# wyysf-98/MoCo_Flow

Measured on AMD Instinct MI355X. Metric: ray-samples/sec (4096 rays x 64 samples), higher is better.
Workload: dtype f32

## Files before the change

include/mocoflow_hip.h:

```cpp
#ifndef MOCOFLOW_HIP_H
#define MOCOFLOW_HIP_H

#include <stdint.h>

#ifdef __cplusplus
extern "C" {
#endif

#define MF_ABI_VERSION 16

enum {
  MF_OK = 0,
  MF_E_INVALID = -1,
  MF_E_LAUNCH = -2,
  MF_E_UNSUPPORTED = -3
};

enum { MF_MAX_FREQS = 16, MF_MAX_LAYERS = 16 };

enum { MF_PREC_F32 = 0, MF_PREC_BF16 = 1, MF_PREC_BF16X3 = 2 };

typedef struct mf_embedding {
  int32_t in_channels;
  int32_t n_freqs;
  float freq[MF_MAX_FREQS];
  float weight[MF_MAX_FREQS];
} mf_embedding;

enum { MF_EXTRA_NONE = 0, MF_EXTRA_IND = 1, MF_EXTRA_DIR = 2 };

typedef struct mf_nerf_desc {
  int32_t D;
  int32_t W;
  int32_t in_channels_xyz;
  uint32_t skip_mask;
  int32_t extra_feat_type;
  int32_t extra_feat_dim;
  const float* trunk_w[MF_MAX_LAYERS];
  const float* trunk_b[MF_MAX_LAYERS];
  const float* final_w; const float* final_b;
  const float* extra_w; const float* extra_b;
  const float* sigma_w; const float* sigma_b;
  const float* rgb_w;   const float* rgb_b;
} mf_nerf_desc;

typedef struct mf_nof_desc {
  int32_t D;
  int32_t W;
  int32_t in_channels_xyz;
  int32_t extra_feat_dim;
  uint32_t skip_mask;
  int32_t use_quat;
  const float* trunk_w[MF_MAX_LAYERS];
  const float* trunk_b[MF_MAX_LAYERS];
  const float* head_w; const float* head_b;
} mf_nof_desc;

int32_t mf_version(void);
const char* mf_last_error(void);

int64_t mf_nerf_packed_bytes(const mf_nerf_desc* d);
int64_t mf_nof_packed_bytes(const mf_nof_desc* d);
int32_t mf_nerf_pack(const mf_nerf_desc* d, void* packed, void* stream);
int32_t mf_nof_pack(const mf_nof_desc* d, void* packed, void* stream);
int64_t mf_nerf_packed_bytes_p(const mf_nerf_desc* d, int32_t precision);
int64_t mf_nof_packed_bytes_p(const mf_nof_desc* d, int32_t precision);
int32_t mf_nerf_pack_p(const mf_nerf_desc* d, int32_t precision, void* packed, void* stream);
int32_t mf_nof_pack_p(const mf_nof_desc* d, int32_t precision, void* packed, void* stream);

int32_t mf_embedding_forward(const mf_embedding* e, const float* x, int64_t B, float* out, void* stream);
int32_t mf_embedding_forward_rows(const mf_embedding* e, const float* x, int64_t B, int32_t repeat, float* out,
                                  int64_t out_stride, void* stream);

int32_t mf_nerf_forward(const mf_nerf_desc* d, const void* packed, const float* inputs,
                        int64_t in_stride, int64_t B, int32_t sigma_only, float* out, void* stream);

int32_t mf_nerf_forward_dump(const mf_nerf_desc* d, const void* packed, const float* inputs, int64_t in_stride,
                             int64_t B, float* out, float* dump_acts, int64_t dump_stride, void* stream);

int32_t mf_nof_forward(const mf_nof_desc* d, const void* packed, const float* inputs,
                       int64_t in_stride, const float* xyz, int64_t B, float* out, void* stream);

int64_t mf_nerf_bwd_packed_bytes(const mf_nerf_desc* d);
int32_t mf_nerf_pack_bwd(const mf_nerf_desc* d, void* packed, void* stream);
int32_t mf_nerf_backward(const mf_nerf_desc* d, const void* packed_bwd, int64_t P, const float* g_out,
                         const float* acts, int64_t stride, const float* rgbsigma, float* gpre,
                         float* ghead, void* stream);

int32_t mf_nerf_backward_x(const mf_nerf_desc* d, const void* packed_bwd, int64_t P, const float* g_out,
                           const float* acts, int64_t stride, const float* rgbsigma, float* gpre,
                           float* ghead, float* g_emb, void* stream);
int64_t mf_nerf_bwd3_packed_bytes(const mf_nerf_desc* d);
int32_t mf_nerf_pack_bwd3(const mf_nerf_desc* d, void* packed, void* stream);
int32_t mf_nerf_backward3(const mf_nerf_desc* d, const void* packed_bwd3, int64_t P, const float* g_out,
                          const float* acts, int64_t stride, const float* rgbsigma, float* gpre,
                          float* ghead, float* g_emb, const uint32_t* mask, int64_t mask_stride, void* stream);
int32_t mf_embedding_backward(const mf_embedding* e, const float* g_emb, int64_t g_stride, const float* emb,
                              int64_t e_stride, int64_t P, float* g_x, void* stream);

int32_t mf_composite_backward(const float* rays, int64_t ray_stride, int64_t n_rays, int32_t S,
                              const float* z_vals, const float* rgbsigma, const float* noise,
                              int32_t activation, const float* background, const float* g_rgb,
                              const float* g_depth, const float* g_opacity, float* g_rgbsigma, void* stream);

#define MF_WG_MAX_ITEMS 32
typedef struct mf_wgrad_item {
  const float* G; int64_t g_stride; int32_t n_out;
  const float* X; int64_t x_stride; int32_t n_in;
  float* dW; float* db;
} mf_wgrad_item;
int64_t mf_weight_grads_scratch_bytes(const mf_wgrad_item* items, int32_t n_items, int64_t P);
int32_t mf_weight_grads(const mf_wgrad_item* items, int32_t n_items, int64_t P, void* scratch, void* stream);
int64_t mf_weight_grads_scratch_bytes_p(int32_t precision, const mf_wgrad_item* items, int32_t n_items, int64_t P);
int32_t mf_weight_grads_p(int32_t precision, const mf_wgrad_item* items, int32_t n_items, int64_t P, void* scratch, void* stream);

int32_t mf_nof_points_dump(const mf_nof_desc* d, const void* packed, const mf_embedding* emb_xyz,
                           const mf_embedding* emb_ind, const float* pts, const float* ind,
                           int64_t ind_stride, int32_t S, int64_t P, float* out, float* acts,
                           int64_t stride, float* emb, void* stream);
int32_t mf_nof_forward_dump(const mf_nof_desc* d, const void* packed, const float* inputs, int64_t in_stride,
                            const float* xyz, int64_t B, float* out, float* acts, int64_t stride, void* stream);
int64_t mf_nof_bwd_packed_bytes(const mf_nof_desc* d);
int32_t mf_nof_pack_bwd(const mf_nof_desc* d, void* packed, void* stream);
int32_t mf_nof_backward(const mf_nof_desc* d, const void* packed_bwd, const mf_embedding* emb_xyz, int64_t P,
                        const float* pts, const float* acts, int64_t stride, const float* g_out,
                        float* gpre, float* g_pts, void* stream);
int64_t mf_nof_bwd3_packed_bytes(const mf_nof_desc* d);
int32_t mf_nof_pack_bwd3(const mf_nof_desc* d, void* packed, void* stream);
int32_t mf_nof_backward3(const mf_nof_desc* d, const void* packed_bwd3, const mf_embedding* emb_xyz, int64_t P,
                         const float* pts, const float* acts, int64_t stride, const float* g_out,
                         float* gpre, float* g_pts, void* stream);

int32_t mf_points_sigma(const mf_nerf_desc* nerf, const void* nerf_packed, const mf_embedding* emb_xyz,
                        const mf_nof_desc* nof, const void* nof_packed, const mf_embedding* nof_emb_xyz,
                        const mf_embedding* nof_emb_ind, const float* xyz, const float* ind,
                        float ind_scalar, int64_t B, float* sigma, float* canon, void* stream);
int32_t mf_points_sigma_p(int32_t precision, const mf_nerf_desc* nerf, const void* nerf_packed, const mf_embedding* emb_xyz,
                          const mf_nof_desc* nof, const void* nof_packed, const mf_embedding* nof_emb_xyz,
                          const mf_embedding* nof_emb_ind, const float* xyz, const float* ind,
                          float ind_scalar, int64_t B, float* sigma, float* canon, void* workspace,
                          int64_t workspace_bytes, void* stream);
int64_t mf_points_sigma_workspace_bytes(int32_t precision, const mf_nof_desc* nof, int32_t per_point_ind, int64_t B);

int32_t mf_points_radiance(const mf_nerf_desc* nerf, const void* nerf_packed, const mf_embedding* emb_xyz,
                           const mf_embedding* emb_extra, const mf_nof_desc* nof, const void* nof_packed,
                           const mf_embedding* nof_emb_xyz, const mf_embedding* nof_emb_ind, const float* xyz,
                           const float* view_dirs, const float* ind, float ind_scalar, int64_t B, float* out,
                           float* canon, void* stream);

enum {
  MF_ACT_RELU = 0, MF_ACT_SOFTPLUS = 1
};
enum {
  MF_F_SIGMA_ONLY   = 1 << 0,
  MF_F_CHAIN_LOCAL  = 1 << 1,
  MF_F_CHAIN_GLOBAL = 1 << 2
};

typedef struct mf_render_args {
  const float* rays; int64_t ray_stride; int64_t n_rays;
  const float* background;
  int32_t n_samples;
  const float* z_vals; const float* z_steps; int32_t use_disp;
  const float* noise;
  int32_t activation;
  int32_t flags;
  const mf_nerf_desc* nerf; const void* nerf_packed;
  mf_embedding emb_xyz;
  mf_embedding emb_extra;
  const mf_nof_desc* nof_bw; const void* nof_bw_packed;
  const mf_nof_desc* nof_fw; const void* nof_fw_packed;
  mf_embedding nof_emb_xyz, nof_emb_ind;
  float* rgb;
  float* depth;
  float* opacity;
  float* weights;
  float* alphas;
  float* disp_local;
  float* disp_global;
  int32_t precision;
  float* dump_acts; int64_t dump_stride;
  float* dump_rgbsigma;
  float* dump_xyz;
  float* dump_nof_acts; int64_t dump_nof_stride;
  float* dump_nof_emb;
  float* dump_nof_out;
  int32_t dump_nof_plane[5];
  void* workspace; int64_t workspace_bytes;
  uint32_t* dump_mask; int64_t dump_mask_stride;
} mf_render_args;

int32_t mf_render_prepare(const mf_render_args* a, void* stream);
int32_t mf_render_pass(const mf_render_args* a, void* stream);
int64_t mf_render_workspace_bytes(const mf_render_args* a);

int32_t mf_nof_emb_slot_features(int32_t* features80);

int32_t mf_nof_embed_rows(const mf_embedding* emb_xyz, const float* pts, const float* ind_emb, int32_t ind_width, int32_t S,
                          int64_t P, float* out, void* stream);

int32_t mf_sample_pdf(const float* bins, const float* z_coarse, const float* weights, int64_t w_stride,
                      int64_t n_rays, int32_t n_bins, int32_t M, const float* u, int64_t u_stride,
                      const float* cdf_in, float* z_new_out, int32_t* inds_out, float* z_sorted_out,
                      void* stream);
int32_t mf_sample_pdf_eps(const float* bins, const float* z_coarse, const float* weights, int64_t w_stride,
                          int64_t n_rays, int32_t n_bins, int32_t M, const float* u, int64_t u_stride,
                          const float* cdf_in, float* z_new_out, int32_t* inds_out, float* z_sorted_out,
                          float eps, void* stream);
int32_t mf_sample_pdf_merge(const float* z_coarse, const float* weights, int64_t n_rays,
                            int32_t S, int32_t M, const float* u, float* z_out,
                            int32_t* inds_out, float* z_new_out, void* stream);

int64_t mf_compact_scratch_bytes(int64_t n_rays);
int32_t mf_compact_mask(const float* alphas, const float* vals_a, const float* vals_b,
                        int64_t n_rays, int32_t S, float* out_a, float* out_b,
                        int64_t* count, void* scratch, void* stream);

typedef struct mf_loss_pass {
  const float* rgb;
  const float* alphas;
  const float* disp_local;
  const float* disp_global;
  int32_t n_samples;
} mf_loss_pass;
int64_t mf_loss_partials_scratch_bytes(void);
int32_t mf_loss_partials(const mf_loss_pass* coarse, const mf_loss_pass* fine, const float* target, int64_t n_rays,
                         double* out12, float* means6, void* scratch, void* stream);

typedef struct mf_loss_grad_pass {
  const float* rgb; float* g_rgb;
  const float* alphas; int32_t n_samples;
  const float* rays; int64_t ray_stride; const float* z_vals;
  const float* recon_local; float* g_recon_local;
  const float* recon_global; float* g_recon_global;
} mf_loss_grad_pass;
int32_t mf_loss_partials_backward(const mf_loss_grad_pass* coarse, const mf_loss_grad_pass* fine, const float* target,
                                  int64_t n_rays, const double* out12, const double* g12, void* stream);

int32_t mf_z_vals(const float* rays, int64_t ray_stride, int64_t n_rays, const float* z_steps, int32_t n_samples,
                  int32_t use_disp, const float* perturb_rand, float perturb, float* z_out, void* stream);

int32_t mf_make_rays(int32_t H, int32_t W, float focal, float cx, float cy, const float* c2w_host,
                     float nearv, float farv, float idx, float* rays_out, void* stream);
int32_t mf_valid_rays_mask(int32_t H, int32_t W, const int32_t* pts_xy_host, int32_t n_pts, uint8_t* mask_out,
                           void* stream);
int32_t mf_image_compose(const uint8_t* rays_msk, const int64_t* rank, int64_t B, const float* opacity,
                         const float* rgb, const float* depth, const float* background, float* img,
                         float* depth_out, void* stream);

int32_t mf_knn1(const float* ref, int64_t V, const float* query, int64_t Q, float* dist, int64_t* ind,
                void* stream);

typedef struct mf_smpl_model {
  int32_t n_verts;
  const float* v_template;
  const float* shapedirs;
  const float* posedirs;
  const float* j_regressor;
  const float* weights;
  int32_t parent[24];
} mf_smpl_model;

int64_t mf_smpl_scratch_bytes(int64_t n_verts, int64_t B);
int32_t mf_smpl_lbs(const mf_smpl_model* m, const float* pose, int32_t pose_is_rotmat, const float* betas, int64_t B,
                    float* verts, float* T, void* scratch, void* stream);

int32_t mf_smpl_frame_transforms(const float* T_src, const float* T_tgt, int64_t V, float* trans, void* stream);

int32_t mf_apply_vertex_transforms(const float* trans, const int64_t* ind, int64_t V, const float* query, int64_t Q,
                                   float* cano, void* stream);

int64_t mf_mc_scratch_bytes(int64_t n0, int64_t n1, int64_t n2);
int32_t mf_mc_count(const float* vol, int64_t n0, int64_t n1, int64_t n2, float iso, int32_t clamp_zero,
                    void* scratch, int64_t* counts, void* stream);
int32_t mf_mc_emit(const float* vol, int64_t n0, int64_t n1, int64_t n2, float iso, int32_t clamp_zero,
                   const void* scratch, float* verts, int64_t* tris, void* stream);
int32_t mf_mc_normals(const float* vol, int64_t n0, int64_t n1, int64_t n2, int32_t clamp_zero, const float* verts, int64_t V,
                      float* normals, void* stream);

int64_t mf_ssim_scratch_bytes(int64_t B, int64_t C, int64_t H, int64_t W);
int32_t mf_ssim(const float* a, const int64_t* a_strides, const float* b, const int64_t* b_strides, int64_t B, int64_t C,
                int64_t H, int64_t W, int32_t window_size, float max_val, float eps, float* map_out, double* sums,
                void* scratch, void* stream);
int64_t mf_sqerr_scratch_bytes(int64_t n);
int32_t mf_sqerr(const float* a, const float* b, int64_t n, const uint8_t* mask, int64_t row_len, double* out2,
                 void* scratch, void* stream);

int64_t mf_depth_range_scratch_bytes(int64_t n);
int32_t mf_depth_range(const float* depth, int64_t n, float nan_value, float* out2, void* scratch, void* stream);
int32_t mf_depth_colormap(const float* depth, int64_t n, const float* range2, float nan_value, const uint8_t* lut,
                          float* out_planar, void* stream);
typedef struct mf_sheet_panel {
  const float* rows;
  int32_t kind;
  float nan_value;
} mf_sheet_panel;
int32_t mf_frame_sheet(const mf_sheet_panel* panels , int32_t n_panels, int64_t H, int64_t W, const float* range2s,
                       const uint8_t* lut, uint8_t* out_u8, float* out_planar, void* stream);

int64_t mf_mask_compact_scratch_bytes(int64_t n);
int32_t mf_mask_compact(const uint8_t* mask, int64_t n, int64_t* inds_out, int64_t* count, void* scratch, void* stream);

enum { MF_IMAGE_NONE = 0, MF_IMAGE_ROWS = 1, MF_IMAGE_U8_RGB = 2, MF_IMAGE_U8_RGBA = 3 };
enum { MF_BACKGROUND_NONE = 0, MF_BACKGROUND_ROWS = 1, MF_BACKGROUND_COLOUR = 2 };
typedef struct mf_ray_batch_args {
  int32_t H, W;
  float focal, cx, cy;
  int32_t has_c2w; float c2w[12];
  float nearv, farv, idx;
  int32_t has_chain; float chain_idx;
  const int64_t* val_inds; int64_t n_valid;
  const int64_t* perm; int64_t n_rows;
  const void* image; int32_t image_kind;
  const float* background; int32_t background_kind;
  float* rays_out; float* rgbs_out; float* background_out; int64_t* sel_out;
} mf_ray_batch_args;
int32_t mf_ray_batch(const mf_ray_batch_args* a , void* stream);

int32_t mf_point_correspond(const float* verts, const float* trans, int64_t V, const float* query, int64_t q_given,
                            const int64_t* pick, const float* noise, int64_t q_near, float thickness, int32_t lanes_per_query,
                            float* pairs, uint8_t* inside, float* dist, int64_t* ind, void* stream);

typedef struct mf_point_loss_args {
  int64_t Q;
  const float* pairs;
  const uint8_t* inside;
  int32_t use_all;
  const float* pred_bw;
  const float* pred_fw;
  int32_t n_nerfs;
  const float* sigma[2];
  float delta[2];
} mf_point_loss_args;
int64_t mf_point_loss_partials_scratch_bytes(int64_t Q);
int32_t mf_point_loss_partials(const mf_point_loss_args* a , double* out6, float* means3, void* scratch, void* stream);

int32_t mf_point_loss_partials_backward(const mf_point_loss_args* a , const double* out6, const float* seeds3,
                                        float* g_pred_bw, float* g_pred_fw, float* g_sigma0, float* g_sigma1, void* stream);

#ifdef __cplusplus
}
#endif
#endif
```

moco_flow_amd/_lib.py:

```python
from __future__ import annotations

import ctypes as C
import os
import threading

MF_MAX_FREQS = 16
MF_MAX_LAYERS = 16
MF_EXTRA_NONE, MF_EXTRA_IND, MF_EXTRA_DIR = 0, 1, 2
MF_ACT_RELU, MF_ACT_SOFTPLUS = 0, 1
MF_F_SIGMA_ONLY, MF_F_CHAIN_LOCAL, MF_F_CHAIN_GLOBAL = 1, 2, 4
MF_PREC_F32, MF_PREC_BF16, MF_PREC_BF16X3 = 0, 1, 2
PRECISIONS = {"f32": MF_PREC_F32, "bf16": MF_PREC_BF16, "bf16x3": MF_PREC_BF16X3}
MF_ABI_VERSION = 16

LIB_PATH = os.environ.get("MOCOFLOW_HIP_LIB") or os.path.join(os.path.dirname(os.path.abspath(__file__)), "libmocoflow_hip.so")

_fp = C.c_void_p


class mf_embedding(C.Structure):
    _fields_ = [("in_channels", C.c_int32), ("n_freqs", C.c_int32),
                ("freq", C.c_float * MF_MAX_FREQS), ("weight", C.c_float * MF_MAX_FREQS)]


class mf_smpl_model(C.Structure):
    _fields_ = [("n_verts", C.c_int32), ("v_template", _fp), ("shapedirs", _fp), ("posedirs", _fp),
                ("j_regressor", _fp), ("weights", _fp), ("parent", C.c_int32 * 24)]


class mf_nerf_desc(C.Structure):
    _fields_ = [("D", C.c_int32), ("W", C.c_int32), ("in_channels_xyz", C.c_int32),
                ("skip_mask", C.c_uint32), ("extra_feat_type", C.c_int32), ("extra_feat_dim", C.c_int32),
                ("trunk_w", _fp * MF_MAX_LAYERS), ("trunk_b", _fp * MF_MAX_LAYERS),
                ("final_w", _fp), ("final_b", _fp), ("extra_w", _fp), ("extra_b", _fp),
                ("sigma_w", _fp), ("sigma_b", _fp), ("rgb_w", _fp), ("rgb_b", _fp)]


class mf_nof_desc(C.Structure):
    _fields_ = [("D", C.c_int32), ("W", C.c_int32), ("in_channels_xyz", C.c_int32),
                ("extra_feat_dim", C.c_int32), ("skip_mask", C.c_uint32), ("use_quat", C.c_int32),
                ("trunk_w", _fp * MF_MAX_LAYERS), ("trunk_b", _fp * MF_MAX_LAYERS),
                ("head_w", _fp), ("head_b", _fp)]


class mf_wgrad_item(C.Structure):
    _fields_ = [("G", _fp), ("g_stride", C.c_int64), ("n_out", C.c_int32),
                ("X", _fp), ("x_stride", C.c_int64), ("n_in", C.c_int32),
                ("dW", _fp), ("db", _fp)]


MF_WG_MAX_ITEMS = 32


class mf_sheet_panel(C.Structure):
    _fields_ = [("rows", _fp), ("kind", C.c_int32), ("nan_value", C.c_float)]


MF_SHEET_MAX_PANELS = 8
MF_PANEL_RGB, MF_PANEL_DEPTH = 0, 1


MF_IMAGE_NONE, MF_IMAGE_ROWS, MF_IMAGE_U8_RGB, MF_IMAGE_U8_RGBA = 0, 1, 2, 3
MF_BACKGROUND_NONE, MF_BACKGROUND_ROWS, MF_BACKGROUND_COLOUR = 0, 1, 2


class mf_ray_batch_args(C.Structure):
    _fields_ = [("H", C.c_int32), ("W", C.c_int32), ("focal", C.c_float), ("cx", C.c_float), ("cy", C.c_float),
                ("has_c2w", C.c_int32), ("c2w", C.c_float * 12), ("nearv", C.c_float), ("farv", C.c_float), ("idx", C.c_float),
                ("has_chain", C.c_int32), ("chain_idx", C.c_float),
                ("val_inds", _fp), ("n_valid", C.c_int64), ("perm", _fp), ("n_rows", C.c_int64),
                ("image", _fp), ("image_kind", C.c_int32), ("background", _fp), ("background_kind", C.c_int32),
                ("rays_out", _fp), ("rgbs_out", _fp), ("background_out", _fp), ("sel_out", _fp)]


class mf_point_loss_args(C.Structure):
    _fields_ = [("Q", C.c_int64), ("pairs", _fp), ("inside", _fp), ("use_all", C.c_int32), ("pred_bw", _fp), ("pred_fw", _fp),
                ("n_nerfs", C.c_int32), ("sigma", _fp * 2), ("delta", C.c_float * 2)]


class mf_loss_pass(C.Structure):
    _fields_ = [("rgb", _fp), ("alphas", _fp), ("disp_local", _fp), ("disp_global", _fp), ("n_samples", C.c_int32)]


class mf_loss_grad_pass(C.Structure):
    _fields_ = [("rgb", _fp), ("g_rgb", _fp), ("alphas", _fp), ("n_samples", C.c_int32),
                ("rays", _fp), ("ray_stride", C.c_int64), ("z_vals", _fp),
                ("recon_local", _fp), ("g_recon_local", _fp), ("recon_global", _fp), ("g_recon_global", _fp)]


class mf_render_args(C.Structure):
    _fields_ = [("rays", _fp), ("ray_stride", C.c_int64), ("n_rays", C.c_int64),
                ("background", _fp), ("n_samples", C.c_int32),
                ("z_vals", _fp), ("z_steps", _fp), ("use_disp", C.c_int32),
                ("noise", _fp), ("activation", C.c_int32), ("flags", C.c_int32),
                ("nerf", C.POINTER(mf_nerf_desc)), ("nerf_packed", _fp),
                ("emb_xyz", mf_embedding), ("emb_extra", mf_embedding),
                ("nof_bw", C.POINTER(mf_nof_desc)), ("nof_bw_packed", _fp),
                ("nof_fw", C.POINTER(mf_nof_desc)), ("nof_fw_packed", _fp),
                ("nof_emb_xyz", mf_embedding), ("nof_emb_ind", mf_embedding),
                ("rgb", _fp), ("depth", _fp), ("opacity", _fp), ("weights", _fp), ("alphas", _fp),
                ("disp_local", _fp), ("disp_global", _fp), ("precision", C.c_int32),
                ("dump_acts", _fp), ("dump_stride", C.c_int64), ("dump_rgbsigma", _fp), ("dump_xyz", _fp),
                ("dump_nof_acts", _fp), ("dump_nof_stride", C.c_int64), ("dump_nof_emb", _fp), ("dump_nof_out", _fp),
                ("dump_nof_plane", C.c_int32 * 5),
                ("workspace", _fp), ("workspace_bytes", C.c_int64),
                ("dump_mask", _fp), ("dump_mask_stride", C.c_int64)]


SYMBOLS = {
    "mf_version": (C.c_int32, []),
    "mf_last_error": (C.c_char_p, []),
    "mf_nerf_packed_bytes": (C.c_int64, [C.POINTER(mf_nerf_desc)]),
    "mf_nof_packed_bytes": (C.c_int64, [C.POINTER(mf_nof_desc)]),
    "mf_nerf_pack": (C.c_int32, [C.POINTER(mf_nerf_desc), _fp, _fp]),
    "mf_nof_pack": (C.c_int32, [C.POINTER(mf_nof_desc), _fp, _fp]),
    "mf_nerf_packed_bytes_p": (C.c_int64, [C.POINTER(mf_nerf_desc), C.c_int32]),
    "mf_nof_packed_bytes_p": (C.c_int64, [C.POINTER(mf_nof_desc), C.c_int32]),
    "mf_nerf_pack_p": (C.c_int32, [C.POINTER(mf_nerf_desc), C.c_int32, _fp, _fp]),
    "mf_nof_pack_p": (C.c_int32, [C.POINTER(mf_nof_desc), C.c_int32, _fp, _fp]),
    "mf_embedding_forward": (C.c_int32, [C.POINTER(mf_embedding), _fp, C.c_int64, _fp, _fp]),
    "mf_embedding_forward_rows": (C.c_int32, [C.POINTER(mf_embedding), _fp, C.c_int64, C.c_int32, _fp, C.c_int64, _fp]),
    "mf_nerf_forward": (C.c_int32, [C.POINTER(mf_nerf_desc), _fp, _fp, C.c_int64, C.c_int64, C.c_int32, _fp, _fp]),
    "mf_nerf_forward_dump": (C.c_int32, [C.POINTER(mf_nerf_desc), _fp, _fp, C.c_int64, C.c_int64, _fp, _fp, C.c_int64, _fp]),
    "mf_nof_forward": (C.c_int32, [C.POINTER(mf_nof_desc), _fp, _fp, C.c_int64, _fp, C.c_int64, _fp, _fp]),
    "mf_nerf_bwd_packed_bytes": (C.c_int64, [C.POINTER(mf_nerf_desc)]),
    "mf_nerf_pack_bwd": (C.c_int32, [C.POINTER(mf_nerf_desc), _fp, _fp]),
    "mf_nof_points_dump": (C.c_int32, [C.POINTER(mf_nof_desc), _fp, C.POINTER(mf_embedding), C.POINTER(mf_embedding), _fp, _fp,
                                       C.c_int64, C.c_int32, C.c_int64, _fp, _fp, C.c_int64, _fp, _fp]),
    "mf_nof_forward_dump": (C.c_int32, [C.POINTER(mf_nof_desc), _fp, _fp, C.c_int64, _fp, C.c_int64, _fp, _fp, C.c_int64, _fp]),
    "mf_nof_bwd_packed_bytes": (C.c_int64, [C.POINTER(mf_nof_desc)]),
    "mf_nof_pack_bwd": (C.c_int32, [C.POINTER(mf_nof_desc), _fp, _fp]),
    "mf_nof_backward": (C.c_int32, [C.POINTER(mf_nof_desc), _fp, C.POINTER(mf_embedding), C.c_int64, _fp, _fp, C.c_int64,
                                    _fp, _fp, _fp, _fp]),
    "mf_nof_backward3": (C.c_int32, [C.POINTER(mf_nof_desc), _fp, C.POINTER(mf_embedding), C.c_int64, _fp, _fp, C.c_int64,
                                    _fp, _fp, _fp, _fp]),
    "mf_nof_bwd3_packed_bytes": (C.c_int64, [C.POINTER(mf_nof_desc)]),
    "mf_nof_pack_bwd3": (C.c_int32, [C.POINTER(mf_nof_desc), _fp, _fp]),
    "mf_composite_backward": (C.c_int32, [_fp, C.c_int64, C.c_int64, C.c_int32, _fp, _fp, _fp, C.c_int32, _fp, _fp, _fp, _fp,
                                          _fp, _fp]),
    "mf_image_compose": (C.c_int32, [_fp, _fp, C.c_int64, _fp, _fp, _fp, _fp, _fp, _fp, _fp]),
    "mf_weight_grads_scratch_bytes": (C.c_int64, [C.POINTER(mf_wgrad_item), C.c_int32, C.c_int64]),
    "mf_weight_grads": (C.c_int32, [C.POINTER(mf_wgrad_item), C.c_int32, C.c_int64, _fp, _fp]),
    "mf_weight_grads_scratch_bytes_p": (C.c_int64, [C.c_int32, C.POINTER(mf_wgrad_item), C.c_int32, C.c_int64]),
    "mf_weight_grads_p": (C.c_int32, [C.c_int32, C.POINTER(mf_wgrad_item), C.c_int32, C.c_int64, _fp, _fp]),
    "mf_nerf_bwd3_packed_bytes": (C.c_int64, [C.POINTER(mf_nerf_desc)]),
    "mf_nerf_pack_bwd3": (C.c_int32, [C.POINTER(mf_nerf_desc), _fp, _fp]),
    "mf_nerf_backward3": (C.c_int32, [C.POINTER(mf_nerf_desc), _fp, C.c_int64, _fp, _fp, C.c_int64, _fp, _fp, _fp, _fp, _fp, C.c_int64, _fp]),
    "mf_nerf_backward": (C.c_int32, [C.POINTER(mf_nerf_desc), _fp, C.c_int64, _fp, _fp, C.c_int64, _fp, _fp, _fp, _fp]),
    "mf_render_pass": (C.c_int32, [C.POINTER(mf_render_args), _fp]),
    "mf_render_workspace_bytes": (C.c_int64, [C.POINTER(mf_render_args)]),
    "mf_render_prepare": (C.c_int32, [C.POINTER(mf_render_args), _fp]),
    "mf_points_sigma_workspace_bytes": (C.c_int64, [C.c_int32, C.POINTER(mf_nof_desc), C.c_int32, C.c_int64]),
    "mf_points_sigma": (C.c_int32, [C.POINTER(mf_nerf_desc), _fp, C.POINTER(mf_embedding), C.POINTER(mf_nof_desc), _fp,
                                    C.POINTER(mf_embedding), C.POINTER(mf_embedding), _fp, _fp, C.c_float, C.c_int64,
                                    _fp, _fp, _fp]),
    "mf_points_sigma_p": (C.c_int32, [C.c_int32, C.POINTER(mf_nerf_desc), _fp, C.POINTER(mf_embedding), C.POINTER(mf_nof_desc), _fp,
                                      C.POINTER(mf_embedding), C.POINTER(mf_embedding), _fp, _fp, C.c_float, C.c_int64,
                                      _fp, _fp, _fp, C.c_int64, _fp]),
    "mf_points_radiance": (C.c_int32, [C.POINTER(mf_nerf_desc), _fp, C.POINTER(mf_embedding), C.POINTER(mf_embedding),
                                       C.POINTER(mf_nof_desc), _fp, C.POINTER(mf_embedding), C.POINTER(mf_embedding), _fp, _fp,
                                       _fp, C.c_float, C.c_int64, _fp, _fp, _fp]),
    "mf_sample_pdf_merge": (C.c_int32, [_fp, _fp, C.c_int64, C.c_int32, C.c_int32, _fp, _fp, _fp, _fp, _fp]),
    "mf_sample_pdf": (C.c_int32, [_fp, _fp, _fp, C.c_int64, C.c_int64, C.c_int32, C.c_int32, _fp, C.c_int64,
                                  _fp, _fp, _fp, _fp, _fp]),
    "mf_sample_pdf_eps": (C.c_int32, [_fp, _fp, _fp, C.c_int64, C.c_int64, C.c_int32, C.c_int32, _fp, C.c_int64,
                                      _fp, _fp, _fp, _fp, C.c_float, _fp]),
    "mf_z_vals": (C.c_int32, [_fp, C.c_int64, C.c_int64, _fp, C.c_int32, C.c_int32, _fp, C.c_float, _fp, _fp]),
    "mf_make_rays": (C.c_int32, [C.c_int32, C.c_int32, C.c_float, C.c_float, C.c_float, C.POINTER(C.c_float),
                                 C.c_float, C.c_float, C.c_float, _fp, _fp]),
    "mf_knn1": (C.c_int32, [_fp, C.c_int64, _fp, C.c_int64, _fp, _fp, _fp]),
    "mf_nof_emb_slot_features": (C.c_int32, [C.POINTER(C.c_int32)]),
    "mf_nof_embed_rows": (C.c_int32, [C.POINTER(mf_embedding), _fp, _fp, C.c_int32, C.c_int32, C.c_int64, _fp, _fp]),
    "mf_smpl_scratch_bytes": (C.c_int64, [C.c_int64, C.c_int64]),
    "mf_smpl_lbs": (C.c_int32, [C.POINTER(mf_smpl_model), _fp, C.c_int32, _fp, C.c_int64, _fp, _fp, _fp, _fp]),
    "mf_smpl_frame_transforms": (C.c_int32, [_fp, _fp, C.c_int64, _fp, _fp]),
    "mf_apply_vertex_transforms": (C.c_int32, [_fp, _fp, C.c_int64, _fp, C.c_int64, _fp, _fp]),
    "mf_nerf_backward_x": (C.c_int32, [C.POINTER(mf_nerf_desc), _fp, C.c_int64, _fp, _fp, C.c_int64, _fp, _fp, _fp, _fp, _fp]),
    "mf_embedding_backward": (C.c_int32, [C.POINTER(mf_embedding), _fp, C.c_int64, _fp, C.c_int64, C.c_int64, _fp, _fp]),
    "mf_valid_rays_mask": (C.c_int32, [C.c_int32, C.c_int32, C.POINTER(C.c_int32), C.c_int32, _fp, _fp]),
    "mf_loss_partials_scratch_bytes": (C.c_int64, []),
    "mf_loss_partials": (C.c_int32, [C.POINTER(mf_loss_pass), C.POINTER(mf_loss_pass), _fp, C.c_int64, _fp, _fp, _fp, _fp]),
    "mf_loss_partials_backward": (C.c_int32, [C.POINTER(mf_loss_grad_pass), C.POINTER(mf_loss_grad_pass), _fp, C.c_int64, _fp, _fp, _fp]),
    "mf_compact_scratch_bytes": (C.c_int64, [C.c_int64]),
    "mf_compact_mask": (C.c_int32, [_fp, _fp, _fp, C.c_int64, C.c_int32, _fp, _fp, _fp, _fp, _fp]),
    "mf_mc_scratch_bytes": (C.c_int64, [C.c_int64, C.c_int64, C.c_int64]),
    "mf_mc_count": (C.c_int32, [_fp, C.c_int64, C.c_int64, C.c_int64, C.c_float, C.c_int32, _fp, _fp, _fp]),
    "mf_mc_emit": (C.c_int32, [_fp, C.c_int64, C.c_int64, C.c_int64, C.c_float, C.c_int32, _fp, _fp, _fp, _fp]),
    "mf_mc_normals": (C.c_int32, [_fp, C.c_int64, C.c_int64, C.c_int64, C.c_int32, _fp, C.c_int64, _fp, _fp]),
    "mf_ssim_scratch_bytes": (C.c_int64, [C.c_int64, C.c_int64, C.c_int64, C.c_int64]),
    "mf_ssim": (C.c_int32, [_fp, C.POINTER(C.c_int64), _fp, C.POINTER(C.c_int64), C.c_int64, C.c_int64, C.c_int64, C.c_int64,
                            C.c_int32, C.c_float, C.c_float, _fp, _fp, _fp, _fp]),
    "mf_sqerr_scratch_bytes": (C.c_int64, [C.c_int64]),
    "mf_sqerr": (C.c_int32, [_fp, _fp, C.c_int64, _fp, C.c_int64, _fp, _fp, _fp]),
    "mf_depth_range_scratch_bytes": (C.c_int64, [C.c_int64]),
    "mf_depth_range": (C.c_int32, [_fp, C.c_int64, C.c_float, _fp, _fp, _fp]),
    "mf_depth_colormap": (C.c_int32, [_fp, C.c_int64, _fp, C.c_float, _fp, _fp, _fp]),
    "mf_frame_sheet": (C.c_int32, [C.POINTER(mf_sheet_panel), C.c_int32, C.c_int64, C.c_int64, _fp, _fp, _fp, _fp, _fp]),
    "mf_mask_compact_scratch_bytes": (C.c_int64, [C.c_int64]),
    "mf_mask_compact": (C.c_int32, [_fp, C.c_int64, _fp, _fp, _fp, _fp]),
    "mf_ray_batch": (C.c_int32, [C.POINTER(mf_ray_batch_args), _fp]),
    "mf_point_correspond": (C.c_int32, [_fp, _fp, C.c_int64, _fp, C.c_int64, _fp, _fp, C.c_int64, C.c_float, C.c_int32,
                                        _fp, _fp, _fp, _fp, _fp]),
    "mf_point_loss_partials_scratch_bytes": (C.c_int64, [C.c_int64]),
    "mf_point_loss_partials": (C.c_int32, [C.POINTER(mf_point_loss_args), _fp, _fp, _fp, _fp]),
    "mf_point_loss_partials_backward": (C.c_int32, [C.POINTER(mf_point_loss_args), _fp, _fp, _fp, _fp, _fp, _fp, _fp]),
}

_lock = threading.Lock()
_lib = None


def lib():
    global _lib
    if _lib is not None:
        return _lib
    with _lock:
        if _lib is None:
            if not os.path.exists(LIB_PATH):
                raise RuntimeError(
                    f"moco_flow_amd: HIP library not built ({LIB_PATH} missing). "
                    "Run `make -C moco_flow_amd/csrc` (hipcc, gfx950). There is no CPU fallback.")
            handle = C.CDLL(LIB_PATH)
            for name, (res, args) in SYMBOLS.items():
                fn = getattr(handle, name)
                fn.restype = res
                fn.argtypes = args
            if handle.mf_version() != MF_ABI_VERSION:
                raise RuntimeError("moco_flow_amd: ABI version mismatch")
            _lib = handle
    return _lib


def check(rc: int, what: str = ""):
    if rc != 0:
        msg = lib().mf_last_error().decode(errors="replace")
        if rc == -3:
            raise NotImplementedError(f"moco_flow_amd HIP path: {msg}")
        raise RuntimeError(f"moco_flow_amd HIP call failed ({what}, rc={rc}): {msg}")


def ptr(t):
    return None if t is None else t.data_ptr()


def current_stream(device) -> int:
    import torch
    return torch.cuda.current_stream(device).cuda_stream


def require_gpu(t, what: str):
    if not t.is_cuda:
        raise RuntimeError(
            f"moco_flow_amd.{what}: tensor is on '{t.device}'. This package is the MI355X (HIP) path and has "
            "no CPU implementation; move the module and its inputs to a 'cuda' device.")
```

moco_flow_amd/csrc/mf_layout.hpp:

```cpp
#pragma once
#include "../../include/mocoflow_hip.h"
#include "mf_core.hpp"

namespace mf {

inline int64_t round_up(int64_t x, int64_t m) { return (x + m - 1) / m * m; }

inline int single_skip_layer(uint32_t skip_mask, int D) {
  int s = 0;
  for (int l = 1; l < D; ++l)
    if ((skip_mask >> l) & 1u) { if (s) return -1; s = l; }
  return s;
}

constexpr int kPackHidden = -1;
struct PackBlock {
  const float* src;
  int s_n, s_k;
  int kind;
  int steps;
  int split;
  int cols;
};

struct PackRegion {
  PackBlock blk[2];
  int tiles;
  int groups;
  int n_rows;
  int row_terms;
  long long dst_group0;
};

struct ResCopy { const float* src; int dst_off; int n; float scale = 1.f; };

struct PackJob {
  PackRegion reg[MF_MAX_LAYERS + 3];
  int n_regions;
  int bf16;
  int xyz_cols;
  int half;
  float wscale;
  long long total_groups;
  float* panels;
  float* poison;
  ResCopy res[2];
  int n_res, res_floats;
  float* resident;
  PackRegion& add(int tiles, int groups, const PackBlock& b0, const PackBlock& b1 = PackBlock{}) {
    PackRegion& R = reg[n_regions++];
    R = PackRegion{{b0, b1}, tiles, groups, 0, 0, total_groups};
    total_groups += (long long)groups * tiles;
    return R;
  }
};
static_assert(sizeof(PackJob) <= 2048, "pack_panels_kernel's argument block");

int launch_pack(const PackJob& job, hipStream_t st, const char* what);

inline bool nerf_layout(const mf_nerf_desc& d, NetLayout& L, int bf16 = 0) {
  L = NetLayout{};
  const bool x3 = bf16 == MF_PREC_BF16X3;
  L.bf16 = bf16 ? 1 : 0;
  if (d.W != 256 && d.W != 128) return false;
  if (d.D < 2 || d.D + 1 > MF_MAX_LAYERS) return false;
  if (d.in_channels_xyz < 3 || d.in_channels_xyz > 64) return false;
  if (d.extra_feat_type != MF_EXTRA_NONE && (d.extra_feat_dim < 1 || d.extra_feat_dim > 32)) return false;
  if (d.skip_mask & 1u) return false;
  if (d.skip_mask >> d.D) return false;
  L.W = d.W;
  L.NK = d.W / 16;
  L.NP = d.W / 32;
  L.n_trunk = d.D + 1;
  if (bf16 && d.W != 256) return false;
  L.emb_steps = bf16 ? kKsNerfXyz : kStepsNerfXyz;
  L.emb_split = x3 ? 1 : 0;
  L.hsplit_mask = x3 ? ((1u << (d.D + 2)) - 1u) & ~1u : 0u;
  L.terms = 2;
  L.emb_mask = 1u | d.skip_mask;
  L.relu_mask = (1u << d.D) - 1u;
  switch (d.extra_feat_type) {
    case MF_EXTRA_NONE: L.extra_steps = 0; break;
    case MF_EXTRA_IND: L.extra_steps = bf16 ? kKsInd : kStepsInd; if (d.extra_feat_dim < 1) return false; break;
    case MF_EXTRA_DIR: L.extra_steps = bf16 ? kKsDir : kStepsDir; if (d.extra_feat_dim < 3) return false; break;
    default: return false;
  }
  int off = 0;
  L.off_bias_trunk = off; off += L.n_trunk * L.W;
  L.off_bias_extra = off; off += L.W / 2;
  L.off_head_w = off; off += L.W;
  L.off_head_b = off; off += 4;
  L.off_rgb_w = off; off += 3 * (L.W / 2);
  L.off_rgb_b = off; off += 4;
  L.n_head = 1;
  L.head_tiles = bf16 == MF_PREC_BF16 ? 1 : 0;
  L.res_bytes = round_up((int64_t)off * 4, kGroupBytes);
  int64_t groups = 0;
  L.max_groups = 0;
  for (int l = 0; l < L.n_trunk; ++l) {
    if (l == L.n_trunk - 1) groups += nerf_sigma_groups(L);
    const int g = trunk_groups(L, l);
    groups += (int64_t)g * L.NP;
    if ((x3 ? panel_cap(g) : g) > L.max_groups) L.max_groups = x3 ? panel_cap(g) : g;
  }
  const int ge = extra_groups(L);
  groups += (int64_t)ge * (L.NP / 2);
  if ((x3 ? panel_cap(ge) : ge) > L.max_groups) L.max_groups = x3 ? panel_cap(ge) : ge;
  groups += nerf_rgb_groups(L);
  L.panel_bytes = groups * kGroupBytes;
  return true;
}

inline bool nof_layout(const mf_nof_desc& d, NetLayout& L, int bf16 = 0, bool wide_ok = false) {
  L = NetLayout{};
  const bool x3 = bf16 == MF_PREC_BF16X3;
  L.bf16 = bf16 ? 1 : 0;
  if (d.W != 128 && !(wide_ok && !bf16 && d.W == 256)) return false;
  if (d.D < 2 || d.D > MF_MAX_LAYERS) return false;
  if (d.in_channels_xyz < 3 || d.in_channels_xyz > 33 || d.extra_feat_dim < 0 || d.extra_feat_dim > 33) return false;
  if ((d.skip_mask & 1u) || (d.skip_mask >> d.D)) return false;
  L.W = d.W;
  L.NK = d.W / 16;
  L.NP = d.W / 32;
  L.n_trunk = d.D;
  L.emb_steps = bf16 ? kKsNofXyz : kStepsNofIn;
  L.emb_split = bf16 ? 1 : 0;
  L.hsplit_mask = x3 ? ((1u << d.D) - 1u) & ~1u : 0u;
  L.terms = x3 ? kNofTermsX3 : 2;
  L.half = (x3 && kNofHalfX3) ? 1 : 0;
  L.head_tiles = bf16 == MF_PREC_BF16 ? 1 : 0;
  L.emb_mask = 1u | d.skip_mask;
  L.relu_mask = (1u << d.D) - 1u;
  L.extra_steps = -1;
  L.n_head = d.use_quat ? 9 : 3;
  int off = 0;
  L.off_bias_trunk = off; off += L.n_trunk * L.W;
  L.off_head_w = off; off += L.n_head * L.W;
  L.off_head_b = off; off += bf16 ? 32 : 12;
  L.res_bytes = round_up((int64_t)off * 4, kGroupBytes);
  int64_t groups = 0;
  L.max_groups = 0;
  for (int l = 0; l < L.n_trunk; ++l) {
    const int g = trunk_groups(L, l);
    groups += (int64_t)g * L.NP;
    if ((x3 ? panel_cap(g) : g) > L.max_groups) L.max_groups = x3 ? panel_cap(g) : g;
  }
  if (bf16) {
    groups += head_groups(L);
    if (head_groups(L) > L.max_groups) L.max_groups = head_groups(L);
  }
  L.panel_bytes = groups * kGroupBytes;
  L.n_emb_layers = __builtin_popcount(L.emb_mask);
  L.ind_bytes = bf16 ? round_up((int64_t)L.n_emb_layers * L.W * kNofIndCols * 4, kGroupBytes) : 0;
  return true;
}

}
```

moco_flow_amd/csrc/mf_nets.hpp:

```cpp
#pragma once
#include "mf_core.hpp"

namespace mf {

MF_D const char* first_panel(const NetDev& n) { return n.packed + n.L.res_bytes; }
MF_D int first_groups(const NetDev& n) { return trunk_groups(n.L, 0); }

MF_D NextLayer follow_of(const NetDev& n) {
  NextLayer f;
  f.groups = trunk_groups(n.L, 0);
  f.jump = n.packed + n.L.res_bytes;
  f.bias_off = n.res_lds + n.L.off_bias_trunk * 4;
  return f;
}
MF_D NextLayer next_trunk(const NetDev& n, int layer) {
  NextLayer f;
  f.groups = trunk_groups(n.L, layer);
  f.jump = nullptr;
  f.bias_off = n.res_lds + (n.L.off_bias_trunk + layer * n.L.W) * 4;
  return f;
}

MF_D void load_resident(const NetDev& n, const LaneId& id) {
  const int groups = (int)(n.L.res_bytes / kGroupBytes);
  for (int g = id.wave; g < groups; g += kWaves) blds16(n.packed, id.lane * 16, g * kGroupBytes, n.res_lds + g * kGroupBytes);
}

template <int PD>
MF_D void start_program(const NetDev& n, Stream& st, CarryT<PD>& carry, const LaneId& id) {
  st.start(first_panel(n), first_groups(n), id);
  carry.load(st.slot_off(0) + id.lane * 16, n.res_lds + n.L.off_bias_trunk * 4, id.g);
}

template <int NK, bool DUMP = false>
MF_D void extra_layer(const NetDev& net, const f32x4 (&act)[NK],
                      const float (&ext)[kStepsExtraMax], f32x4 (&out)[NK / 2],
                      Stream& st, CarryT<kPD>& carry, const LaneId& id, const NextLayer& nxt,
                      float* dump_row = nullptr, unsigned* mask_row = nullptr) {
  constexpr int NPO = NK / 4;
  constexpr int QH = NK;
  const int groups = extra_groups(net.L);
  const int qe = net.L.extra_steps / 4;
  const uint32_t bias_off = net.res_lds + net.L.off_bias_extra * 4;
  const float dummy[4] = {0.f, 0.f, 0.f, 0.f};
  static_assert(NPO % 4 == 0, "mask words collect four panels");
  unsigned macc = 0;
#pragma unroll
  for (int t = 0; t < NPO; ++t) {
    const uint32_t p = st.slot_off(0) + id.lane * 16;
    const uint32_t pn = st.slot_off(1) + id.lane * 16;
    const uint32_t nb = (t + 1 < NPO) ? bias_off + 32 * (t + 1) * 4 : nxt.bias_off;
    auto hook = [&](int ph) { st.template sync_and_dma<DUMP>(t + 2 < NPO ? groups : nxt.groups, t == NPO - 2 ? nxt.jump : nullptr, id, ph); };
    f32x4 E, O;
    out_pair<2, NK, 4>(carry, act, dummy, p, pn, nb, id.g, id.wave < kWaves / 2 && !(st.dbg & 64), hook,
                             -__builtin_inff(), E, O);
#pragma unroll
    for (int q = 0; q < kStepsExtraMax / 4; ++q) {
      if (q < qe) {
        const f32x4 wE = lds_f4(p + (2 * (QH + q)) * kGroupBytes);
        const f32x4 wO = lds_f4(p + (2 * (QH + q) + 1) * kGroupBytes);
#pragma unroll
        for (int r = 0; r < 4; ++r) {
          E = MF_MFMA(wE[r], ext[4 * q + r], E);
          O = MF_MFMA(wO[r], ext[4 * q + r], O);
        }
      }
    }
#pragma unroll
    for (int i = 0; i < 4; ++i) {
      E[i] = fmaxf(E[i], 0.f);
      O[i] = fmaxf(O[i], 0.f);
    }
    out[2 * t] = E;
    out[2 * t + 1] = O;
    if constexpr (DUMP) {
      if (dump_row) {
        *reinterpret_cast<f32x4*>(dump_row + 32 * t + 4 * id.g) = E;
        *reinterpret_cast<f32x4*>(dump_row + 32 * t + 16 + 4 * id.g) = O;
      }
      const bool wm = __ballot(mask_row != nullptr) != 0ull;
      const bool put = wm && relu_mask_put(macc, mask_row, dump_row && mask_row, t, id.g, E, O);
      st.keep2 = __ballot(dump_row != nullptr) != 0ull ? (put ? 3 : 2) : 0;
    }
    st.advance();
  }
}

template <int NK, bool DUMP = false>
MF_D void nerf_eval(const NetDev& net, const float (&embx)[kStepsNerfXyz], const float (&ext)[kStepsExtraMax],
                    bool sigma_only, Stream& st, CarryT<kPD>& carry, const LaneId& id,
                    const NextLayer& follow, float& sigma, float (&rgb)[3], float* dump_row = nullptr,
                    unsigned* mask_row = nullptr) {
  f32x4 act[NK];
#pragma unroll
  for (int t = 0; t < NK; ++t)
#pragma unroll
    for (int i = 0; i < 4; ++i) act[t][i] = 0;
  const int D = net.L.n_trunk - 1;
  for (int l = 0; l < D; ++l) {
    const bool last = sigma_only && l == D - 1;
    trunk_layer<NK, kStepsNerfXyz, DUMP>(net, l, act, embx, st, carry, id, last ? follow : next_trunk(net, l + 1),
                                               dump_row ? dump_row + l * net.L.W : nullptr, mask_row ? mask_row + l * 8 : nullptr);
    st.tl.stamp(10 + l, id);
  }
  float sg[1];
  valu_head(act, net.res_lds + net.L.off_head_w * 4, net.L.W, net.res_lds + net.L.off_head_b * 4, id.g, sg);
  sigma = sg[0];
  st.tl.stamp(30, id);
  if (sigma_only) return;
  NextLayer ex;
  ex.groups = extra_groups(net.L);
  ex.jump = nullptr;
  ex.bias_off = net.res_lds + net.L.off_bias_extra * 4;
  trunk_layer<NK, kStepsNerfXyz, DUMP>(net, D, act, embx, st, carry, id, ex,
                                             dump_row ? dump_row + D * net.L.W : nullptr);
  st.tl.stamp(31, id);
  f32x4 e[NK / 2];
  extra_layer<NK, DUMP>(net, act, ext, e, st, carry, id, follow, dump_row ? dump_row + (D + 1) * net.L.W : nullptr,
                        mask_row ? mask_row + (D + 1) * 8 : nullptr);
  st.tl.stamp(33, id);
  float o[3];
  valu_head(e, net.res_lds + net.L.off_rgb_w * 4, net.L.W / 2, net.res_lds + net.L.off_rgb_b * 4, id.g, o);
#pragma unroll
  for (int c = 0; c < 3; ++c) rgb[c] = 1.f / (1.f + expf(-o[c]));
}

template <bool FAST = false>
MF_D void quat_transform(const float (&T)[9], const float (&xyz)[3], float (&out)[3]) {
  const float vx = T[0], vy = T[1], vz = T[2];
  float qx, qy, qz, qw;
  if constexpr (FAST) {
    const float n = fmaxf(__builtin_amdgcn_sqrtf(vx * vx + vy * vy + vz * vz), 1e-8f);
    const float rev = n * 0.15915494309189535f;
    const float s_n = __builtin_amdgcn_sinf(rev) * __builtin_amdgcn_rcpf(n);
    qx = vx * s_n; qy = vy * s_n; qz = vz * s_n; qw = __builtin_amdgcn_cosf(rev);
    const float rq = __builtin_amdgcn_rcpf(fmaxf(__builtin_amdgcn_sqrtf(qx * qx + qy * qy + qz * qz + qw * qw), 1e-12f));
    qx *= rq; qy *= rq; qz *= rq; qw *= rq;
  } else {
    float n = sqrtf(vx * vx + vy * vy + vz * vz);
    n = fmaxf(n, 1e-8f);
    float sn, cn;
    sincosf(n, &sn, &cn);
    qx = vx * sn / n; qy = vy * sn / n; qz = vz * sn / n; qw = cn;
    const float qn = fmaxf(sqrtf(qx * qx + qy * qy + qz * qz + qw * qw), 1e-12f);
    qx /= qn; qy /= qn; qz /= qn; qw /= qn;
  }
  const float tx = 2.f * qx, ty = 2.f * qy, tz = 2.f * qz;
  const float twx = tx * qw, twy = ty * qw, twz = tz * qw;
  const float txx = tx * qx, txy = ty * qx, txz = tz * qx;
  const float tyy = ty * qy, tyz = tz * qy, tzz = tz * qz;
  const float R00 = 1.f - (tyy + tzz), R01 = txy - twz, R02 = txz + twy;
  const float R10 = txy + twz, R11 = 1.f - (txx + tzz), R12 = tyz - twx;
  const float R20 = txz - twy, R21 = tyz + twx, R22 = 1.f - (txx + tyy);
  const float px = xyz[0] - T[3], py = xyz[1] - T[4], pz = xyz[2] - T[5];
  out[0] = (px * R00 + py * R10 + pz * R20) + T[3] + T[6];
  out[1] = (px * R01 + py * R11 + pz * R21) + T[4] + T[7];
  out[2] = (px * R02 + py * R12 + pz * R22) + T[5] + T[8];
}

template <bool DUMP = false, int NK = 8>
MF_D void nof_eval(const NetDev& net, const float (&emb)[kStepsNofIn], const float (&xyz)[3], Stream& st,
                   CarryT<kPD>& carry, const LaneId& id, const NextLayer& follow, float (&out)[3],
                   float* drow = nullptr, bool masks = false) {
  static_assert(!DUMP || NK == 8, "the dump layout (bit rows: four words per layer) is the 128-wide one");
  f32x4 act[NK];
#pragma unroll
  for (int t = 0; t < NK; ++t)
#pragma unroll
    for (int i = 0; i < 4; ++i) act[t][i] = 0;
  const int D = net.L.n_trunk;
  for (int l = 0; l < D; ++l) {
    const bool last = l == D - 1;
    trunk_layer<NK, kStepsNofIn, DUMP>(net, l, act, emb, st, carry, id, last ? follow : next_trunk(net, l + 1),
                                       drow ? drow + l * net.L.W : nullptr,
                                       (DUMP && drow && masks) ? reinterpret_cast<unsigned*>(drow + D * net.L.W + 16) + 4 * l : nullptr);
  }
  const uint32_t wo = net.res_lds + net.L.off_head_w * 4, bo = net.res_lds + net.L.off_head_b * 4;
  float T[9] = {0.f, 0.f, 0.f, 0.f, 0.f, 0.f, 0.f, 0.f, 0.f};
  if (net.L.n_head == 9) {
    valu_head(act, wo, net.L.W, bo, id.g, T);
    quat_transform(T, xyz, out);
  } else {
    float T3[3];
    valu_head(act, wo, net.L.W, bo, id.g, T3);
#pragma unroll
    for (int c = 0; c < 3; ++c) { T[c] = T3[c]; out[c] = T3[c] + xyz[c]; }
  }
  if constexpr (DUMP) {
    if (drow && id.g == 0) {
      float4* tr = reinterpret_cast<float4*>(drow + D * net.L.W);
      tr[0] = make_float4(T[0], T[1], T[2], T[3]);
      tr[1] = make_float4(T[4], T[5], T[6], T[7]);
      tr[2] = make_float4(T[8], 0.f, 0.f, 0.f);
      tr[3] = make_float4(0.f, 0.f, 0.f, 0.f);
    }
  }
}

MF_D void nof_embed(float (&emb)[kStepsNofIn], const float (&xyz)[3], float ind, const EmbParams& exyz,
                    const EmbParams& eind, int g) {
  emb_eval<3, 5>(emb, xyz, exyz, g);
  const float iv[1] = {ind};
  emb_eval<1, 16>(emb + BlkXyz5::SLOTS, iv, eind, g);
#pragma unroll
  for (int e = BlkXyz5::SLOTS + BlkInd16::SLOTS; e < kStepsNofIn; ++e) emb[e] = 0.f;
}

MF_D void nof_embed_lds(float (&emb)[kStepsNofIn], const float (&xyz)[3], float ind, uint32_t par_xyz, uint32_t par_ind, int g) {
  emb_eval_lds<3, 5>(emb, xyz, par_xyz, g);
  const float iv[1] = {ind};
  emb_eval_lds<1, 16>(emb + BlkXyz5::SLOTS, iv, par_ind, g);
#pragma unroll
  for (int e = BlkXyz5::SLOTS + BlkInd16::SLOTS; e < kStepsNofIn; ++e) emb[e] = 0.f;
}

}
```

moco_flow_amd/csrc/mf_pack.hip:

```cpp
#include <hip/hip_fp16.h>
#include "mf_host.hpp"
#include "mf_layout.hpp"

namespace mf {

__device__ inline unsigned short bf16_rne(float x) {
  const unsigned u = __float_as_uint(x);
  const unsigned rnd = u + 0x7fffu + ((u >> 16) & 1u);
  return (unsigned short)(((u & 0x7f800000u) == 0x7f800000u ? u : rnd) >> 16);
}

__device__ inline float resident_value(const ResCopy* c, int n, int idx) {
  float v = 0.f;
  for (int k = 0; k < n; ++k) {
    const int o = idx - c[k].dst_off;
    if (o >= 0 && o < c[k].n) v = c[k].src[o] * c[k].scale;
  }
  return v;
}

__device__ inline float block_at(const PackBlock& B, int n, int c) {
  return (c >= 0 && c < B.cols) ? B.src[(long long)n * B.s_n + (long long)c * B.s_k] : 0.f;
}

__global__ void pack_panels_kernel(PackJob job) {
  const long long gidx = (long long)blockIdx.x * blockDim.x + threadIdx.x;
  if (gidx < job.res_floats) job.resident[gidx] = resident_value(job.res, job.n_res, (int)gidx);
  const long long grp = ((long long)blockIdx.x * blockDim.x + __builtin_amdgcn_readfirstlane(threadIdx.x)) >> 6;
  if (grp >= job.total_groups) return;
  const int lane = (int)(gidx & 63);
  int ri = 0;
  while (ri + 1 < job.n_regions && grp >= job.reg[ri + 1].dst_group0) ++ri;
  const PackRegion& R = job.reg[ri];
  const long long local = grp - R.dst_group0;
  const int P = (int)(local / R.groups), gi = (int)(local % R.groups);
  float4 v = make_float4(0.f, 0.f, 0.f, 0.f);
  float* pv = &v.x;
  if (job.bf16) {
    const int i = lane & 31, h = lane >> 5;
    int srow = 32 * P + i, rterm = 0;
    bool zero_row = R.n_rows && srow >= R.n_rows;
    if (R.row_terms) {
      zero_row = !(srow < R.n_rows || (srow >= R.row_terms && srow < R.row_terms + R.n_rows));
      if (srow >= R.row_terms) { rterm = 1; srow -= R.row_terms; }
    }
    const int g0 = R.blk[0].split * R.blk[0].steps;
    const PackBlock B = gi < g0 ? R.blk[0] : R.blk[1];
    const int gb = gi < g0 ? gi : gi - g0;
    unsigned short h8[8] = {0, 0, 0, 0, 0, 0, 0, 0};
    const bool half = job.half != 0;
    const float ws = job.wscale;
    bool sat = false;
    auto term = [half, ws, &sat](float w, int t) {
      if (half) {
        w = w * ws;
        if (!(fabsf(w) <= 65504.f)) sat = true;
        w = fminf(fmaxf(w, -65504.f), 65504.f);
        __half hb = __float2half_rn(w);
        if (t > 0) hb = __float2half_rn(w - __half2float(hb));
        return __half_as_ushort(hb);
      }
      unsigned short b = bf16_rne(w);
      for (int k = 0; k < t; ++k) {
        w -= __uint_as_float((unsigned)b << 16);
        b = bf16_rne(w);
      }
      return b;
    };
    if (!zero_row && gb < B.split * B.steps) {
      const int ks = gb / B.split, t = R.row_terms ? rterm : gb % B.split;
#pragma unroll
      for (int e = 0; e < 8; ++e) {
        const int c = B.kind == kPackHidden ? 16 * ks + hid_perm2(h, e) : emb_feature2(B.kind, h, 8 * ks + e, job.xyz_cols);
        h8[e] = term(block_at(B, srow, c), t);
      }
    }
    unsigned* pu = reinterpret_cast<unsigned*>(&v.x);
    for (int w = 0; w < 4; ++w) pu[w] = (unsigned)h8[2 * w] | ((unsigned)h8[2 * w + 1] << 16);
    reinterpret_cast<float4*>(job.panels)[gidx] = v;
    if (sat && job.poison) { job.poison[0] = __int_as_float(0x7fc00000); job.poison[4] = __int_as_float(0x7fc00000); }
    return;
  }
  const int b = gi >> 1, half = gi & 1;
  const int i = lane & 15, g = lane >> 4;
  const int n = 32 * P + 16 * half + i;
  const PackBlock B = b < R.blk[0].steps ? R.blk[0] : R.blk[1];
  const int q = b < R.blk[0].steps ? b : b - R.blk[0].steps;
  if (!(R.n_rows && n >= R.n_rows) && q < B.steps)
#pragma unroll
    for (int r = 0; r < 4; ++r)
      pv[r] = block_at(B, n, B.kind == kPackHidden ? 16 * q + 4 * g + r : emb_feature(B.kind, g, 4 * q + r, job.xyz_cols));
  reinterpret_cast<float4*>(job.panels)[gidx] = v;
}

struct ResJob { ResCopy c[2 * MF_MAX_LAYERS + 8]; int n; float* res; int total; };

__global__ void pack_resident_kernel(ResJob job) {
  const int idx = blockIdx.x * blockDim.x + threadIdx.x;
  if (idx >= job.total) return;
  job.res[idx] = resident_value(job.c, job.n, idx);
}

struct IndJob { const float* W[MF_MAX_LAYERS]; int n_in[MF_MAX_LAYERS]; int n_layers, rows, col0, cols; float* dst; float scale; };

__global__ void pack_ind_kernel(IndJob job) {
  const int idx = blockIdx.x * blockDim.x + threadIdx.x;
  const int per_layer = job.rows * kNofIndCols;
  if (idx >= job.n_layers * per_layer) return;
  const int e = idx / per_layer, r = (idx % per_layer) / kNofIndCols, c = idx % kNofIndCols;
  job.dst[(e * kNofIndCols + c) * job.rows + r] = c < job.cols ? job.scale * job.W[e][(long long)r * job.n_in[e] + job.col0 + c] : 0.f;
}

int launch_pack(const PackJob& job, hipStream_t st, const char* what) {
  const long long slots = job.total_groups * 64 > job.res_floats ? job.total_groups * 64 : job.res_floats;
  hipLaunchKernelGGL(pack_panels_kernel, dim3((unsigned)((slots + 255) / 256)), dim3(256), 0, st, job);
  return check_launch(what);
}

static int launch_pack(const PackJob& job, const ResJob& rj, hipStream_t st) {
  hipLaunchKernelGGL(pack_resident_kernel, dim3((rj.total + 255) / 256), dim3(256), 0, st, rj);
  return launch_pack(job, st, "mf_pack");
}

}

using namespace mf;

extern "C" int64_t mf_nerf_packed_bytes_p(const mf_nerf_desc* d, int32_t precision) {
  NetLayout L;
  if (!d || (precision < MF_PREC_F32 || precision > MF_PREC_BF16X3) || !nerf_layout(*d, L, precision)) { fail(MF_E_UNSUPPORTED, "mf_nerf_packed_bytes: unsupported NeRF configuration"); return 0; }
  return L.res_bytes + L.panel_bytes;
}

extern "C" int64_t mf_nof_packed_bytes_p(const mf_nof_desc* d, int32_t precision) {
  NetLayout L;
  if (!d || (precision < MF_PREC_F32 || precision > MF_PREC_BF16X3) || !nof_layout(*d, L, precision, precision == MF_PREC_F32)) { fail(MF_E_UNSUPPORTED, "mf_nof_packed_bytes: unsupported NoF configuration"); return 0; }
  return L.res_bytes + L.panel_bytes + L.ind_bytes;
}

extern "C" int32_t mf_nerf_pack_p(const mf_nerf_desc* d, int32_t precision, void* packed, void* stream) {
  NetLayout L;
  if (!d || !packed) return fail(MF_E_INVALID, "mf_nerf_pack: null argument");
  if (precision < MF_PREC_F32 || precision > MF_PREC_BF16X3) return fail(MF_E_INVALID, "mf_nerf_pack: precision %d", precision);
  if (!nerf_layout(*d, L, precision)) return fail(MF_E_UNSUPPORTED, "mf_nerf_pack: unsupported NeRF configuration "
                                       "(W=%d D=%d in_channels_xyz=%d)", d->W, d->D, d->in_channels_xyz);
  PackJob job{};
  ResJob rj{};
  const int esplit = L.emb_split ? L.terms : 1, equad = L.bf16 ? 1 : 4;
  auto head_region = [&](const float* W, int rows, int groups) {
    PackRegion& R = job.add(1, groups, PackBlock{W, groups * 16, 1, kPackHidden, groups, 1, groups * 16});
    R.n_rows = rows;
    R.row_terms = 8;
  };
  for (int l = 0; l < L.n_trunk; ++l) {
    if (l == L.n_trunk - 1 && L.head_tiles) {
      if (!d->sigma_w) return fail(MF_E_INVALID, "mf_nerf_pack: missing sigma weight");
      head_region(d->sigma_w, 1, nerf_sigma_groups(L));
    }
    const bool has_emb = (L.emb_mask >> l) & 1;
    const float* W = l < d->D ? d->trunk_w[l] : d->final_w;
    if (!W) return fail(MF_E_INVALID, "mf_nerf_pack: missing weight pointer for layer %d", l);
    const int hid0 = has_emb ? d->in_channels_xyz : 0, n_in = hid0 + (l > 0 ? L.W : 0);
    job.add(L.NP, trunk_groups(L, l),
            PackBlock{W, n_in, 1, kEmbNerfXyz, has_emb ? L.emb_steps / equad : 0, esplit, d->in_channels_xyz},
            PackBlock{W + hid0, n_in, 1, kPackHidden, l > 0 ? hidden_batches(L) : 0, ((L.hsplit_mask >> l) & 1) ? L.terms : 1, L.W});
    const float* b = l < d->D ? d->trunk_b[l] : d->final_b;
    rj.c[rj.n++] = ResCopy{b, L.off_bias_trunk + l * L.W, L.W};
  }
  {
    const int ext = d->extra_feat_type == MF_EXTRA_NONE ? 0 : d->extra_feat_dim;
    const float* W = d->extra_w;
    if (!W) return fail(MF_E_INVALID, "mf_nerf_pack: missing extra_encoding weight");
    const int kind = d->extra_feat_type == MF_EXTRA_DIR ? kEmbDir : (d->extra_feat_type == MF_EXTRA_IND ? kEmbInd : kEmbNone);
    job.add(L.NP / 2, extra_groups(L),
            PackBlock{W, L.W + ext, 1, kPackHidden, hidden_batches(L), ((L.hsplit_mask >> L.n_trunk) & 1) ? L.terms : 1, L.W},
            PackBlock{W + L.W, L.W + ext, 1, kind, L.extra_steps / equad, esplit, ext});
    rj.c[rj.n++] = ResCopy{d->extra_b, L.off_bias_extra, L.W / 2};
  }
  if (L.head_tiles) {
    if (!d->rgb_w) return fail(MF_E_INVALID, "mf_nerf_pack: missing rgb weight");
    head_region(d->rgb_w, 3, nerf_rgb_groups(L));
  }
  rj.c[rj.n++] = ResCopy{d->sigma_w, L.off_head_w, L.W};
  rj.c[rj.n++] = ResCopy{d->sigma_b, L.off_head_b, 1};
  rj.c[rj.n++] = ResCopy{d->rgb_w, L.off_rgb_w, 3 * (L.W / 2)};
  rj.c[rj.n++] = ResCopy{d->rgb_b, L.off_rgb_b, 3};
  for (int k = 0; k < rj.n; ++k)
    if (!rj.c[k].src) return fail(MF_E_INVALID, "mf_nerf_pack: missing bias/head pointer (%d)", k);
  job.bf16 = L.bf16;
  job.xyz_cols = d->in_channels_xyz;
  job.panels = reinterpret_cast<float*>(static_cast<char*>(packed) + L.res_bytes);
  rj.res = static_cast<float*>(packed);
  rj.total = (int)(L.res_bytes / 4);
  if (job.total_groups * kGroupBytes != L.panel_bytes) return fail(MF_E_INVALID, "mf_nerf_pack: layout mismatch");
  return launch_pack(job, rj, static_cast<hipStream_t>(stream));
}

extern "C" int32_t mf_nof_pack_p(const mf_nof_desc* d, int32_t precision, void* packed, void* stream) {
  NetLayout L;
  if (!d || !packed) return fail(MF_E_INVALID, "mf_nof_pack: null argument");
  if (precision < MF_PREC_F32 || precision > MF_PREC_BF16X3) return fail(MF_E_INVALID, "mf_nof_pack: precision %d", precision);
  if (!nof_layout(*d, L, precision, precision == MF_PREC_F32)) return fail(MF_E_UNSUPPORTED, "mf_nof_pack: unsupported NoF configuration "
                                      "(W=%d D=%d in_channels_xyz=%d extra_feat_dim=%d)", d->W, d->D,
                                      d->in_channels_xyz, d->extra_feat_dim);
  PackJob job{};
  ResJob rj{};
  const int cin = d->in_channels_xyz + d->extra_feat_dim;
  const float wscale = L.half ? (float)(1 << kNofHalfSW) : 1.f, bscale = L.half ? (float)(1 << (kNofHalfSA + kNofHalfSW)) : 1.f;
  const int esplit = L.emb_split ? L.terms : 1, equad = L.bf16 ? 1 : 4;
  for (int l = 0; l < L.n_trunk; ++l) {
    const bool has_emb = (L.emb_mask >> l) & 1;
    const float* W = d->trunk_w[l];
    if (!W || !d->trunk_b[l]) return fail(MF_E_INVALID, "mf_nof_pack: missing parameter pointer for layer %d", l);
    const int hid0 = has_emb ? cin : 0, n_in = hid0 + (l > 0 ? L.W : 0);
    job.add(L.NP, trunk_groups(L, l),
            PackBlock{W, n_in, 1, kEmbNofIn, has_emb ? L.emb_steps / equad : 0, esplit, cin},
            PackBlock{W + hid0, n_in, 1, kPackHidden, l > 0 ? hidden_batches(L) : 0, ((L.hsplit_mask >> l) & 1) ? L.terms : 1, L.W});
    rj.c[rj.n++] = ResCopy{d->trunk_b[l], L.off_bias_trunk + l * L.W, L.W, bscale};
  }
  if (!d->head_w || !d->head_b) return fail(MF_E_INVALID, "mf_nof_pack: missing head parameters");
  if (L.bf16) {
    PackRegion& R = job.add(1, head_groups(L), PackBlock{d->head_w, L.W, 1, kPackHidden, L.NK, L.head_tiles ? 1 : L.terms, L.W});
    R.n_rows = L.n_head;
    R.row_terms = L.head_tiles ? 16 : 0;
  }
  rj.c[rj.n++] = ResCopy{d->head_w, L.off_head_w, L.n_head * L.W};
  rj.c[rj.n++] = ResCopy{d->head_b, L.off_head_b, L.n_head, bscale};
  job.bf16 = L.bf16;
  job.xyz_cols = d->in_channels_xyz;
  job.half = L.half;
  job.wscale = wscale;
  job.panels = reinterpret_cast<float*>(static_cast<char*>(packed) + L.res_bytes);
  job.poison = L.half ? static_cast<float*>(packed) + L.off_head_b + 27 : nullptr;
  rj.res = static_cast<float*>(packed);
  rj.total = (int)(L.res_bytes / 4);
  if (job.total_groups * kGroupBytes != L.panel_bytes) return fail(MF_E_INVALID, "mf_nof_pack: layout mismatch");
  if (L.bf16) {
    IndJob ij{};
    for (int l = 0; l < L.n_trunk; ++l)
      if ((L.emb_mask >> l) & 1) {
        ij.W[ij.n_layers] = d->trunk_w[l];
        ij.n_in[ij.n_layers] = cin + (l > 0 ? L.W : 0);
        ++ij.n_layers;
      }
    ij.rows = L.W; ij.col0 = d->in_channels_xyz; ij.cols = d->extra_feat_dim;
    ij.scale = bscale;
    ij.dst = reinterpret_cast<float*>(static_cast<char*>(packed) + L.res_bytes + L.panel_bytes);
    const int total = ij.n_layers * ij.rows * kNofIndCols;
    hipLaunchKernelGGL(pack_ind_kernel, dim3((total + 255) / 256), dim3(256), 0, static_cast<hipStream_t>(stream), ij);
  }
  return launch_pack(job, rj, static_cast<hipStream_t>(stream));
}

extern "C" int64_t mf_nerf_packed_bytes(const mf_nerf_desc* d) { return mf_nerf_packed_bytes_p(d, MF_PREC_F32); }
extern "C" int64_t mf_nof_packed_bytes(const mf_nof_desc* d) { return mf_nof_packed_bytes_p(d, MF_PREC_F32); }
extern "C" int32_t mf_nerf_pack(const mf_nerf_desc* d, void* packed, void* stream) { return mf_nerf_pack_p(d, MF_PREC_F32, packed, stream); }
extern "C" int32_t mf_nof_pack(const mf_nof_desc* d, void* packed, void* stream) { return mf_nof_pack_p(d, MF_PREC_F32, packed, stream); }
```

moco_flow_amd/csrc/mf_render.hip:

```cpp
#include <cstddef>

#include "mf_host.hpp"
#include "mf_layout.hpp"
#include "mf_nets.hpp"
#include "mf_plan.hpp"
#include "mf_raypass.hpp"

namespace mf {

struct RenderParams {
  const float* rays; long long ray_stride; long long n_rays;
  const float* bg;
  int S;
  const float* z_vals; const float* z_steps; int use_disp;
  const float* noise;
  int activation, flags;
  NetDev nerf;
  int extra_type;
  NetDev bw, fw;
  float emb_par[4][32];
  uint32_t par_off;
  float *rgb, *depth, *opacity, *weights, *alphas, *disp_local, *disp_global;
  int G;
  long long n_groups;
  uint32_t ring_off, buf_bytes, sbuf_off, zbuf_off;
  int dbg;
  float* dump_acts; long long dump_stride; float* dump_rgbsigma; float* dump_xyz;
  unsigned* dump_mask; long long dump_mask_stride;
  float* dump_nof_acts; long long dump_nof_stride; float* dump_nof_emb; float* dump_nof_out;
  uint32_t nof_plane_pack;
};

template <bool MOCO, bool DUMP>
__global__ __launch_bounds__(kThreads, 2) void render_kernel(RenderParams p) {
  const LaneId id;
  const NetDev nerf = p.nerf;
  const WgClock wg;
  load_resident(nerf, id);
  if (MOCO) {
    load_resident(p.bw, id);
    if (p.flags & (MF_F_CHAIN_LOCAL | MF_F_CHAIN_GLOBAL)) load_resident(p.fw, id);
  }
  emb_tables_to_lds(p);
  const uint32_t par_nerf_xyz = p.par_off, par_nerf_ext = p.par_off + 128, par_nof_xyz = p.par_off + 256,
                 par_nof_ind = p.par_off + 384;
  Stream st;
  CarryT<kPD> carry;
  st.open(p.ring_off, p.buf_bytes, MF_TIMING_FLAGS ? p.dbg : 0);
  st.tl.start(p.alphas, id);
  const NextLayer prog_first = MOCO ? follow_of(p.bw) : follow_of(nerf);
  if (MOCO) start_program(p.bw, st, carry, id);
  else start_program(nerf, st, carry, id);

  const int S = p.S;
  const bool sigma_only = p.flags & MF_F_SIGMA_ONLY;
  float4* sbuf = reinterpret_cast<float4*>(smem + p.sbuf_off);
  float* zbuf = reinterpret_cast<float*>(smem + p.zbuf_off);

  for (long long group = blockIdx.x; group < p.n_groups; group += gridDim.x) {
    const long long ray0 = group * p.G;
    const int nr = (int)((p.n_rays - ray0) < p.G ? (p.n_rays - ray0) : p.G);
    const int nsamp = nr * S;
    const int ntiles = (nsamp + kTile - 1) / kTile;

    for (int tile = 0; tile < ntiles; ++tile) {
      st.tl.stamp(1, id);
      struct Where { int srel, sl, si; bool valid; long long ray; const float* rp; };
      auto where = [&]() {
        int jo = id.j;
        asm volatile("" : "+v"(jo));
        Where w;
        w.srel = tile * kTile + id.wave * kWaveSamples + jo;
        w.valid = w.srel < nsamp;
        w.sl = w.valid ? w.srel : nsamp - 1;
        const int rr = w.sl / S;
        w.si = w.sl - rr * S;
        w.ray = ray0 + rr;
        w.rp = p.rays + w.ray * p.ray_stride;
        return w;
      };
      float xin[3];
      {
        const Where w = where();
        const float* rp = w.rp;
        const float o[3] = {rp[0], rp[1], rp[2]};
        const float d[3] = {rp[3], rp[4], rp[5]};
        const float z = ray_depth(p, rp, w.ray, w.si);
        ray_point(o, d, z, xin);
        if (w.valid && id.g == 0) {
          zbuf[w.srel] = z;
          if (MOCO) sbuf[w.srel] = make_float4(xin[0], xin[1], xin[2], 0.f);
        }
      }
#ifdef MF_TIMELINE
      asm volatile("s_waitcnt vmcnt(0)" : "+v"(xin[0]), "+v"(xin[1]), "+v"(xin[2]));
#endif
      st.tl.stamp(2, id);
      if (MOCO) {
        const int nsteps = chain_steps(p.flags);
        float canon[3] = {0.f, 0.f, 0.f}, cur[3] = {xin[0], xin[1], xin[2]};
        for (int step = 0; step < nsteps; ++step) {
          const int role = step;
          const NetDev net = role_uses_fw(role) ? p.fw : p.bw;
          const Where w = where();
          const float ind = w.rp[role_ind_column(role)];
          if (role == 1 || role == 2) { cur[0] = canon[0]; cur[1] = canon[1]; cur[2] = canon[2]; }
          const bool last = step == nsteps - 1;
          const NextLayer follow = last ? follow_of(nerf) : (role_uses_fw(role + 1) ? follow_of(p.fw) : follow_of(p.bw));
          float emb[kStepsNofIn], out[3];
          nof_embed_lds(emb, cur, ind, par_nof_xyz, par_nof_ind, id.g);
          float* nof_row = nullptr;
          if constexpr (DUMP) {
            if (w.valid && p.dump_nof_acts) {
              const long long nof_idx = (long long)((p.nof_plane_pack >> (3 * step)) & 7u) * p.n_rays * S + (w.ray * S + w.si);
              nof_row = p.dump_nof_acts + nof_idx * p.dump_nof_stride;
              float4* e4 = reinterpret_cast<float4*>(p.dump_nof_emb + nof_idx * 80 + 20 * id.g);
#pragma unroll
              for (int q = 0; q < kStepsNofIn / 4; ++q) e4[q] = make_float4(emb[4 * q], emb[4 * q + 1], emb[4 * q + 2], emb[4 * q + 3]);
            }
            st.keep2 = 0;
          }
          nof_eval<DUMP>(net, emb, cur, st, carry, id, follow, out, nof_row,
                         DUMP && p.dump_nof_stride >= (long long)net.L.n_trunk * net.L.W + 16 + 4 * net.L.n_trunk);
          if constexpr (DUMP) {
            const Where v = where();
            if (v.valid && p.dump_nof_acts && id.g == 0) {
              const long long nof_idx = (long long)((p.nof_plane_pack >> (3 * step)) & 7u) * p.n_rays * S + (v.ray * S + v.si);
              float* q = p.dump_nof_out + nof_idx * 3;
              q[0] = out[0]; q[1] = out[1]; q[2] = out[2];
            }
          }
          if (role == 0) { canon[0] = out[0]; canon[1] = out[1]; canon[2] = out[2]; }
          if (role == 1 || role == 4) {
            const Where v = where();
            const float4 x4 = sbuf[v.sl];
            const float dd = (fabsf(x4.x - out[0]) + fabsf(x4.y - out[1]) + fabsf(x4.z - out[2])) / 3.f;
            float* plane = role == 1 ? p.disp_local : p.disp_global;
            if (v.valid && id.g == 0 && plane) plane[v.ray * S + v.si] = dd;
          }
          cur[0] = out[0]; cur[1] = out[1]; cur[2] = out[2];
        }
        xin[0] = canon[0]; xin[1] = canon[1]; xin[2] = canon[2];
      }

      st.tl.stamp(3, id);
      float embx[kStepsNerfXyz], ext[kStepsExtraMax];
      if (!(MF_TIMING_FLAGS && (p.dbg & 4))) emb_eval_lds<3, 10>(embx, xin, par_nerf_xyz, id.g);
      else { for (int e = 0; e < kStepsNerfXyz; ++e) embx[e] = xin[e % 3]; }
#pragma unroll
      for (int e = BlkXyz10::SLOTS; e < kStepsNerfXyz; ++e) embx[e] = 0.f;
#pragma unroll
      for (int e = 0; e < kStepsExtraMax; ++e) ext[e] = 0.f;
      float* dump_row = nullptr;
      unsigned* mask_row = nullptr;
      {
        const Where w = where();
        if (!sigma_only) {
          if (p.extra_type == MF_EXTRA_DIR) {
            const float dd[3] = {w.rp[3], w.rp[4], w.rp[5]};
            emb_eval_lds<3, 4>(ext, dd, par_nerf_ext, id.g);
          } else if (p.extra_type == MF_EXTRA_IND) {
            const float iv[1] = {w.rp[8]};
            emb_eval_lds<1, 2>(ext, iv, par_nerf_ext, id.g);
          }
        }
        if constexpr (DUMP) {
          if (w.valid && p.dump_acts) dump_row = p.dump_acts + (w.ray * S + w.si) * p.dump_stride;
          if (p.dump_mask) mask_row = p.dump_mask + (w.ray * S + w.si) * p.dump_mask_stride;
        }
      }
      st.tl.stamp(4, id);
      float sigma, rgb[3] = {0.f, 0.f, 0.f};
      st.keep2 = 0;
      nerf_eval<16, DUMP>(nerf, embx, ext, sigma_only, st, carry, id, prog_first, sigma, rgb, dump_row, mask_row);
      {
        const Where w = where();
        if (w.valid && id.g == 0) {
          sbuf[w.srel] = make_float4(rgb[0], rgb[1], rgb[2], sigma);
          if constexpr (DUMP) {
            const long long row = w.ray * S + w.si;
            if (p.dump_rgbsigma) *reinterpret_cast<float4*>(p.dump_rgbsigma + row * 4) = make_float4(rgb[0], rgb[1], rgb[2], sigma);
            if (p.dump_xyz) { float* q = p.dump_xyz + row * 3; q[0] = xin[0]; q[1] = xin[1]; q[2] = xin[2]; }
          }
        }
      }
      st.tl.stamp(5, id);
    }
    __syncthreads();
    st.tl.stamp(6, id);

    composite_group<kWaves>(p, id.lane, id.wave, ray0, (MF_TIMING_FLAGS && (p.dbg & 8)) ? 0 : nr, S, sigma_only, sbuf, zbuf);
    st.tl.stamp(7, id);
    __syncthreads();
    st.tl.stamp(8, id);
  }
  wait_vm0();
  wg.stamp(p);
}

int render_pass_bf16(const mf_render_args* a, hipStream_t st, bool prepare_only);
int64_t render_workspace_bytes_bf16(const mf_render_args* a);

}

using namespace mf;

extern "C" int64_t mf_render_workspace_bytes(const mf_render_args* a) {
  if (!a || (a->precision != MF_PREC_BF16 && a->precision != MF_PREC_BF16X3) || a->n_rays <= 0) return 0;
  return render_workspace_bytes_bf16(a);
}

extern "C" int32_t mf_nof_emb_slot_features(int32_t* features80) {
  if (!features80) return fail(MF_E_INVALID, "mf_nof_emb_slot_features: null argument");
  for (int g = 0; g < 4; ++g)
    for (int e = 0; e < kStepsNofIn; ++e) features80[kStepsNofIn * g + e] = emb_feature(kEmbNofIn, g, e, 33);
  return MF_OK;
}

static int32_t check_render_args(const mf_render_args* a, NetLayout (&L)[3]) {
  if (!a->rays || a->ray_stride < 9) return fail(MF_E_INVALID, "mf_render_pass: rays missing or ray_stride < 9");
  if (!a->z_vals && !a->z_steps) return fail(MF_E_INVALID, "mf_render_pass: need z_vals or z_steps");
  if (a->activation != MF_ACT_RELU && a->activation != MF_ACT_SOFTPLUS)
    return fail(MF_E_INVALID, "mf_render_pass: activation %d not supported", a->activation);
  if (a->precision < MF_PREC_F32 || a->precision > MF_PREC_BF16X3)
    return fail(MF_E_INVALID, "mf_render_pass: precision %d", a->precision);
  if (!nerf_layout(*a->nerf, L[0], 0)) return fail(MF_E_UNSUPPORTED, "mf_render_pass: unsupported NeRF configuration");
  if (L[0].NK != 16) return fail(MF_E_UNSUPPORTED, "mf_render_pass: only W=256 NeRF is built");
  const bool dump = a->dump_acts || a->dump_rgbsigma || a->dump_xyz || a->dump_nof_acts;
  if (dump && a->precision == MF_PREC_BF16)
    return fail(MF_E_UNSUPPORTED, "mf_render_pass: the activation dump (training forward) exists in fp32 and in bf16x3");
  if (int e = check_xyz_embedding("mf_render_pass", a->emb_xyz, 10)) return e;
  const bool sigma_only = a->flags & MF_F_SIGMA_ONLY;
  if (!sigma_only && a->nerf->extra_feat_type == MF_EXTRA_DIR &&
      (a->emb_extra.in_channels != 3 || a->emb_extra.n_freqs > 4 ||
       3 * (2 * a->emb_extra.n_freqs + 1) > a->nerf->extra_feat_dim))
    return fail(MF_E_UNSUPPORTED, "mf_render_pass: dir embedding must have 3 channels, <= 4 frequencies and fit extra_feat_dim");
  if (!sigma_only && a->nerf->extra_feat_type == MF_EXTRA_IND &&
      (a->emb_extra.in_channels != 1 || a->emb_extra.n_freqs > 2 ||
       (2 * a->emb_extra.n_freqs + 1) > a->nerf->extra_feat_dim))
    return fail(MF_E_UNSUPPORTED, "mf_render_pass: ind embedding must have 1 channel, <= 2 frequencies and fit extra_feat_dim");
  const bool moco = a->nof_bw != nullptr;
  const bool chains = a->flags & (MF_F_CHAIN_LOCAL | MF_F_CHAIN_GLOBAL);
  if (!moco && chains) return fail(MF_E_INVALID, "mf_render_pass: chain flags need NoF models");
  if ((a->flags & MF_F_CHAIN_GLOBAL) && !(a->flags & MF_F_CHAIN_LOCAL))
    return fail(MF_E_INVALID, "mf_render_pass: chain_global without chain_local (the reference raises UnboundLocalError, rendering.py:276-280)");
  if ((a->flags & MF_F_CHAIN_GLOBAL) && a->ray_stride < 10)
    return fail(MF_E_INVALID, "mf_render_pass: chain_global needs the chained image index column (ray_stride >= 10)");
  if (moco) {
    if (!a->nof_bw_packed) return fail(MF_E_INVALID, "mf_render_pass: nof_bw_packed missing");
    if (!nof_layout(*a->nof_bw, L[1], 0)) return fail(MF_E_UNSUPPORTED, "mf_render_pass: unsupported backward NoF configuration");
    if (chains) {
      if (!a->nof_fw || !a->nof_fw_packed) return fail(MF_E_INVALID, "mf_render_pass: chain flags need the forward NoF");
      if (!nof_layout(*a->nof_fw, L[2], 0)) return fail(MF_E_UNSUPPORTED, "mf_render_pass: unsupported forward NoF configuration");
    }
    if (int e = check_nof_embeddings("mf_render_pass", a->nof_emb_xyz, a->nof_emb_ind)) return e;
  }
  return MF_OK;
}

static int32_t render_pass_f32(const mf_render_args* a, const NetLayout (&L)[3], hipStream_t st) {
  const bool moco = a->nof_bw != nullptr;
  const bool chains = a->flags & (MF_F_CHAIN_LOCAL | MF_F_CHAIN_GLOBAL);
  RenderParams p{};
  fill_render_io(p, a);
  p.dbg = debug_flags();
  LdsPlan plan;
  auto place = [&](NetDev& n, const NetLayout& l, const void* packed) { n.L = l; plan.place(n, packed); };
  place(p.nerf, L[0], a->nerf_packed);
  emb_table(a->emb_xyz, p.emb_par[0], p.emb_par[0] + 16);
  emb_table(a->emb_extra, p.emb_par[1], p.emb_par[1] + 16);
  if (moco) {
    place(p.bw, L[1], a->nof_bw_packed);
    if (chains) place(p.fw, L[2], a->nof_fw_packed);
    emb_table(a->nof_emb_xyz, p.emb_par[2], p.emb_par[2] + 16);
    emb_table(a->nof_emb_ind, p.emb_par[3], p.emb_par[3] + 16);
  }
  p.par_off = plan.place_tables();
  plan.ring(p.ring_off, p.buf_bytes);
  uint32_t lds = plan.lds;

  if (int e = plan_ray_groups(a->n_rays, a->n_samples, kTile, lds, p.G, p.n_groups)) return e;
  place_sample_buffers(p, lds);

  if (int e = check_dump_rows(a, p.nerf.L)) return e;
  if (int e = check_dump_mask(a, p.nerf.L)) return e;
  if (a->dump_nof_acts) {
    if (!moco || !a->dump_nof_emb || !a->dump_nof_out) return fail(MF_E_INVALID, "mf_render_pass: dump_nof_acts needs NoF models, dump_nof_emb and dump_nof_out");
    if (a->dump_nof_stride < (int64_t)p.bw.L.n_trunk * p.bw.L.W + 16 || (a->dump_nof_stride & 3))
      return fail(MF_E_INVALID, "mf_render_pass: dump_nof_stride %lld invalid", (long long)a->dump_nof_stride);
    if (a->nof_fw && (p.fw.L.n_trunk != p.bw.L.n_trunk || p.fw.L.W != p.bw.L.W))
      return fail(MF_E_UNSUPPORTED, "mf_render_pass: NoF dumps need bw and fw of the same depth and width");
    if (int e = nof_plane_pack(a, p.nof_plane_pack)) return e;
  }
  p.dump_nof_acts = a->dump_nof_acts; p.dump_nof_stride = a->dump_nof_stride; p.dump_nof_emb = a->dump_nof_emb; p.dump_nof_out = a->dump_nof_out;
  const bool dump = a->dump_acts || a->dump_rgbsigma || a->dump_xyz || a->dump_nof_acts;
  void (*kern)(RenderParams) =
      dump ? (moco ? render_kernel<true, true> : render_kernel<false, true>)
           : (moco ? render_kernel<true, false> : render_kernel<false, false>);
  return launch_lds(kern, persistent_grid(p.n_groups), kThreads, lds, st, p, "mf_render_pass", "mf_render_pass");
}

static int32_t render_entry(const mf_render_args* a, void* stream, bool prepare_only) {
  if (!a || !a->nerf || !a->nerf_packed) return fail(MF_E_INVALID, "mf_render_pass: null argument");
  if (a->n_rays < 0 || a->n_samples < 1) return fail(MF_E_INVALID, "mf_render_pass: n_rays=%lld n_samples=%d", (long long)a->n_rays, a->n_samples);
  if (a->n_rays == 0) return MF_OK;
  NetLayout L[3];
  if (int e = check_render_args(a, L)) return e;
  if (a->precision != MF_PREC_F32) return render_pass_bf16(a, static_cast<hipStream_t>(stream), prepare_only);
  return prepare_only ? MF_OK : render_pass_f32(a, L, static_cast<hipStream_t>(stream));
}
extern "C" int32_t mf_render_pass(const mf_render_args* a, void* stream) { return render_entry(a, stream, false); }
extern "C" int32_t mf_render_prepare(const mf_render_args* a, void* stream) { return render_entry(a, stream, true); }
```

moco_flow_amd/nerf.py:

```python
import torch
from torch import nn

from . import _lib as L
from .packing import PackedWeights


class NeRF(nn.Module):

    def __init__(self, D=8, W=256, in_channels_xyz=33, skips=[4], extra_feat_type="none", extra_feat_dim=0):
        super().__init__()
        self.D = D
        self.W = W
        self.in_channels_xyz = in_channels_xyz
        self.skips = skips
        for i in range(D):
            if i == 0:
                layer = nn.Linear(in_channels_xyz, W)
            elif i in skips:
                layer = nn.Linear(W + in_channels_xyz, W)
            else:
                layer = nn.Linear(W, W)
            setattr(self, f"xyz_encoding_{i+1}", nn.Sequential(layer, nn.ReLU(True)))
        self.xyz_encoding_final = nn.Linear(W, W)
        self.extra_feat_type = extra_feat_type
        self.extra_feat_dim = extra_feat_dim
        assert extra_feat_type in ["none", "ind", "dir", "latent_code"], \
            f"extra_feat_type {extra_feat_type} for NeRF model not supported!!!"
        if extra_feat_type != "none":
            if extra_feat_type == "latent_code":
                self.app_code = torch.randn(1000, extra_feat_dim, requires_grad=True)
            self.extra_encoding = nn.Sequential(nn.Linear(W + extra_feat_dim, W // 2), nn.ReLU(True))
        else:
            self.extra_encoding = nn.Sequential(nn.Linear(W, W // 2), nn.ReLU(True))
        self.sigma = nn.Linear(W, 1)
        self.rgb = nn.Sequential(nn.Linear(W // 2, 3), nn.Sigmoid())
        self._packed = PackedWeights()
        self._packed_bf16 = PackedWeights()
        self._packed_x3 = PackedWeights()
        self._packed_bwd3 = PackedWeights()
        self._packed_bwd = PackedWeights()

    def _build_desc(self):
        if self.extra_feat_type == "latent_code":
            raise NotImplementedError("NeRF model does not support latent code yet!!!")
        d = L.mf_nerf_desc()
        d.D, d.W, d.in_channels_xyz = self.D, self.W, self.in_channels_xyz
        mask = 0
        for s in self.skips:
            if 0 <= s < self.D:
                mask |= 1 << s
        d.skip_mask = mask
        d.extra_feat_type = {"none": L.MF_EXTRA_NONE, "ind": L.MF_EXTRA_IND, "dir": L.MF_EXTRA_DIR}[self.extra_feat_type]
        d.extra_feat_dim = self.extra_feat_dim
        keep = []

        def dp(t):
            t = t.detach().contiguous().float()
            keep.append(t)
            return t.data_ptr()

        if self.D + 1 > L.MF_MAX_LAYERS:
            raise NotImplementedError(f"NeRF with D={self.D} is not built (max {L.MF_MAX_LAYERS - 1})")
        for i in range(self.D):
            lin = getattr(self, f"xyz_encoding_{i+1}")[0]
            d.trunk_w[i], d.trunk_b[i] = dp(lin.weight), dp(lin.bias)
        d.final_w, d.final_b = dp(self.xyz_encoding_final.weight), dp(self.xyz_encoding_final.bias)
        d.extra_w, d.extra_b = dp(self.extra_encoding[0].weight), dp(self.extra_encoding[0].bias)
        d.sigma_w, d.sigma_b = dp(self.sigma.weight), dp(self.sigma.bias)
        d.rgb_w, d.rgb_b = dp(self.rgb[0].weight), dp(self.rgb[0].bias)
        return d, keep

    def packed(self, precision=L.MF_PREC_F32):
        lib = L.lib()
        cache = {L.MF_PREC_F32: self._packed, L.MF_PREC_BF16: self._packed_bf16, L.MF_PREC_BF16X3: self._packed_x3}[precision]
        return cache.get(self, self._build_desc, lib.mf_nerf_packed_bytes_p, lib.mf_nerf_pack_p, "NeRF", precision)

    def invalidate_packed(self):
        for c in (self._packed, self._packed_bf16, self._packed_x3, self._packed_bwd, self._packed_bwd3):
            c.invalidate()

    def packed_bwd(self):
        lib = L.lib()
        return self._packed_bwd.get(self, self._build_desc, lambda d, _p: lib.mf_nerf_bwd_packed_bytes(d),
                                    lambda d, _p, buf, st: lib.mf_nerf_pack_bwd(d, buf, st), "NeRF backward", "bwd")

    def packed_bwd3(self):
        lib = L.lib()
        return self._packed_bwd3.get(self, self._build_desc, lambda d, _p: lib.mf_nerf_bwd3_packed_bytes(d),
                                     lambda d, _p, buf, st: lib.mf_nerf_pack_bwd3(d, buf, st), "NeRF backward (bf16x3)", "bwd3")

    def forward(self, inputs, sigma_only=False, img_ind=None):
        L.require_gpu(inputs, "NeRF.forward")
        if sigma_only:
            width = self.in_channels_xyz
        else:
            width = self.in_channels_xyz + self.extra_feat_dim
        if inputs.dim() != 2 or inputs.shape[1] != width:
            raise RuntimeError(f"NeRF.forward expects (B, {width}) [in_channels_xyz={self.in_channels_xyz}, "
                               f"extra_feat_dim={self.extra_feat_dim}, sigma_only={sigma_only}], "
                               f"got {tuple(inputs.shape)}")
        from . import autograd as A
        want_grad = A.needs_grad([self]) or (torch.is_grad_enabled() and inputs.requires_grad)
        if want_grad and inputs.shape[0] > 0:
            if not A.nerf_fused_eligible(self, inputs.shape[0]):
                raise NotImplementedError(f"NeRF.forward with gradients: the HIP backward is built for W = 256, one xyz block of <= 64 "
                                          f"columns and an extra block of <= 32 (got W={self.W}, in_channels_xyz={self.in_channels_xyz}, "
                                          f"extra_feat_dim={self.extra_feat_dim}, skips={self.skips}); there is no eager fallback")
            return A.NerfModule.apply(self, inputs, bool(sigma_only), *self.parameters())
        desc, buf = self.packed()
        x = inputs.detach().float()
        if x.stride(1) != 1:
            x = x.contiguous()
        B = x.shape[0]
        out = torch.empty((B, 1 if sigma_only else 4), device=x.device, dtype=torch.float32)
        with torch.cuda.device(x.device):
            L.check(L.lib().mf_nerf_forward(desc, buf.data_ptr(), L.ptr(x), x.stride(0) if B else width, B,
                                            1 if sigma_only else 0, L.ptr(out), L.current_stream(x.device)),
                    "mf_nerf_forward")
        return out
```

moco_flow_amd/rendering.py:

```python
from __future__ import annotations

import ctypes as C

import torch

from . import _lib as L
from . import autograd as A
from .packing import BuildOrder

PRECISION = "f32"
TRAIN_FORWARD_PRECISION = "f32"


def set_train_forward_precision(p: str):
    global TRAIN_FORWARD_PRECISION
    if p not in ("f32", "bf16x3"):
        raise ValueError(f"training-forward precision must be 'f32' or 'bf16x3', got {p!r}")
    TRAIN_FORWARD_PRECISION = p


def set_precision(p: str):
    global PRECISION
    if p not in L.PRECISIONS:
        raise ValueError(f"precision must be one of {sorted(L.PRECISIONS)}, got {p!r}")
    PRECISION = p




LAZY_CONSENSUS = True
FUSED_CONSENSUS_MEAN = True


STRICT_RNG = True


_LINSPACE = {}


def _linspace01(S, dev):
    key = (S, str(dev))
    hit = _LINSPACE.get(key)
    if hit is None:
        order = BuildOrder(dev)
        hit = _LINSPACE[key] = (torch.linspace(0, 1, S, device=dev), order)
    else:
        hit[1].order(dev)
    return hit[0]


def _emb_desc(e):
    return e.descriptor() if e is not None else L.mf_embedding()


def _render_pass(rays, background, z_vals, z_steps, use_disp, noise, activation, nerf, nerf_embs,
                 nof_models, nof_embs, chain_local, chain_global, sigma_only, want_planes, dump=False, precision=None,
                 workspace=None):
    dev = rays.device
    N = rays.shape[0]
    S = z_vals.shape[1] if z_vals is not None else z_steps.shape[0]
    extra_emb = nerf_embs[1] if nerf.extra_feat_type == "ind" else (nerf_embs[2] if nerf.extra_feat_type == "dir" else None)
    if nerf_embs[0].out_channels > nerf.in_channels_xyz or \
            (extra_emb is not None and not sigma_only and extra_emb.out_channels > nerf.extra_feat_dim):
        raise RuntimeError(f"render_rays: embedding wider than the NeRF's input block (xyz {nerf_embs[0].out_channels} > "
                           f"{nerf.in_channels_xyz} or {nerf.extra_feat_type} > {nerf.extra_feat_dim})")
    if nof_models is not None:
        for m in nof_models[:2 if (chain_local or chain_global) else 1]:
            if nof_embs[0].out_channels > m.in_channels_xyz or nof_embs[1].out_channels != m.extra_feat_dim:
                raise RuntimeError(f"render_rays: the NoF takes [xyz <= {m.in_channels_xyz} | ind = {m.extra_feat_dim}] input columns, "
                                   f"the embeddings give {nof_embs[0].out_channels} | {nof_embs[1].out_channels}")
    a = L.mf_render_args()
    a.rays, a.ray_stride, a.n_rays = L.ptr(rays), rays.stride(0), N
    a.background = L.ptr(background)
    a.n_samples = S
    a.z_vals, a.z_steps, a.use_disp = L.ptr(z_vals), L.ptr(z_steps), 1 if use_disp else 0
    a.noise = L.ptr(noise)
    a.activation = activation
    flags = 0
    if sigma_only:
        flags |= L.MF_F_SIGMA_ONLY
    if chain_local:
        flags |= L.MF_F_CHAIN_LOCAL
    if chain_global:
        flags |= L.MF_F_CHAIN_GLOBAL
    a.flags = flags
    prec = L.PRECISIONS[precision or PRECISION]
    a.precision = prec
    desc, buf = nerf.packed(prec)
    a.nerf, a.nerf_packed = C.pointer(desc), buf.data_ptr()
    a.emb_xyz = _emb_desc(nerf_embs[0])
    if nerf.extra_feat_type == "ind":
        a.emb_extra = _emb_desc(nerf_embs[1])
    elif nerf.extra_feat_type == "dir":
        a.emb_extra = _emb_desc(nerf_embs[2])
    keep = [desc, buf]
    if nof_models is not None:
        bd, bb = nof_models[0].packed(prec)
        a.nof_bw, a.nof_bw_packed = C.pointer(bd), bb.data_ptr()
        keep += [bd, bb]
        if chain_local or chain_global:
            fd, fb = nof_models[1].packed(prec)
            a.nof_fw, a.nof_fw_packed = C.pointer(fd), fb.data_ptr()
            keep += [fd, fb]
        a.nof_emb_xyz, a.nof_emb_ind = _emb_desc(nof_embs[0]), _emb_desc(nof_embs[1])
    out = {}

    def alloc(name, shape, cond=True):
        if cond:
            out[name] = torch.empty(shape, device=dev, dtype=torch.float32)
            return out[name].data_ptr()
        return None

    a.rgb = alloc("rgb", (N, 3), not sigma_only)
    a.depth = alloc("depth", (N,), not sigma_only)
    a.opacity = alloc("opacity", (N,))
    a.weights = alloc("weights", (N, S), want_planes)
    a.alphas = alloc("alphas", (N, S), want_planes)
    a.disp_local = alloc("disp_local", (N, S), chain_local)
    a.disp_global = alloc("disp_global", (N, S), chain_global)
    if dump:
        stride = (nerf.D + 1) * nerf.W + nerf.W // 2
        a.dump_acts = alloc("acts", (N * S, stride), not sigma_only)
        a.dump_stride = stride
        a.dump_rgbsigma = alloc("rgbsig", (N * S, 4))
        a.dump_xyz = alloc("xyz_in", (N * S, 3))
        if not sigma_only and prec in (L.MF_PREC_F32, L.MF_PREC_BF16X3) and A.DX_PRECISION == "bf16x3":
            mw = (nerf.D + 2) * 8
            out["acts"]._mf_mask = torch.empty((N * S, mw), device=dev, dtype=torch.int32)
            a.dump_mask, a.dump_mask_stride = out["acts"]._mf_mask.data_ptr(), mw
        if nof_models is not None and len({(m.D, m.W) for m in nof_models}) == 1:
            steps = 1 + (1 if chain_local else 0) + (3 if chain_global else 0)
            order = [k for k in range(steps) if k in (0, 3)] + [k for k in range(steps) if k in (1, 2, 4)]
            out["nof_plane"] = [order.index(k) for k in range(steps)]
            for k in range(steps):
                a.dump_nof_plane[k] = out["nof_plane"][k]
            x3 = prec == L.MF_PREC_BF16X3
            nstride = A.nof_dump_stride(nof_models[0])
            a.dump_nof_acts = alloc("nof_acts", (steps, N * S, nstride))
            a.dump_nof_stride = nstride
            if x3:
                out["nof_emb"] = None
            else:
                a.dump_nof_emb = alloc("nof_emb", (steps, N * S, 80))
            a.dump_nof_out = alloc("nof_out", (steps, N * S, 3))
    need = int(L.lib().mf_render_workspace_bytes(C.byref(a)))
    with torch.cuda.device(dev):
        if need > 0:
            shared = workspace if workspace is not None else [None]
            fresh = shared[0] is None or shared[0].numel() < need
            if fresh:
                shared[0] = torch.empty(need, dtype=torch.uint8, device=dev)
            a.workspace, a.workspace_bytes = shared[0].data_ptr(), need
            keep.append(shared[0])
            if fresh:
                L.check(L.lib().mf_render_prepare(C.byref(a), L.current_stream(dev)), "mf_render_prepare")
        L.check(L.lib().mf_render_pass(C.byref(a), L.current_stream(dev)), "mf_render_pass")
    del keep
    return out


def _loss_partials_hip(c, f, target, N):
    dev = target.device
    lib = L.lib()
    tgt = target.detach().contiguous().float()
    if tgt.shape != (N, 3):
        raise RuntimeError(f"_loss_target must be (N, 3) = ({N}, 3), got {tuple(tgt.shape)}")

    def desc(p):
        d = L.mf_loss_pass()
        d.rgb = L.ptr(p.get("rgb"))
        planes = p.get("disp_local") is not None or p.get("disp_global") is not None
        d.alphas = L.ptr(p.get("alphas")) if planes else None
        d.disp_local, d.disp_global = L.ptr(p.get("disp_local")), L.ptr(p.get("disp_global"))
        d.n_samples = p["alphas"].shape[1] if planes else 0
        return d

    dc = desc(c)
    df = desc(f) if f is not None else None
    out = torch.empty(12, dtype=torch.float64, device=dev)
    scratch = torch.empty(int(lib.mf_loss_partials_scratch_bytes()), dtype=torch.uint8, device=dev)
    with torch.cuda.device(dev):
        L.check(lib.mf_loss_partials(C.byref(dc), C.byref(df) if df is not None else None, tgt.data_ptr(), N,
                                     out.data_ptr(), None, scratch.data_ptr(), L.current_stream(dev)), "mf_loss_partials")
    return out


def _compact(alphas, vals_a, vals_b):
    dev = alphas.device
    N, S = alphas.shape
    lib = L.lib()
    scratch = torch.empty(int(lib.mf_compact_scratch_bytes(N)), dtype=torch.uint8, device=dev)
    count = torch.zeros(1, dtype=torch.int64, device=dev)
    oa = torch.empty(N * S, device=dev, dtype=torch.float32) if vals_a is not None else None
    ob = torch.empty(N * S, device=dev, dtype=torch.float32) if vals_b is not None else None
    with torch.cuda.device(dev):
        L.check(lib.mf_compact_mask(L.ptr(alphas), L.ptr(vals_a), L.ptr(vals_b), N, S, L.ptr(oa), L.ptr(ob),
                                    count.data_ptr(), scratch.data_ptr(), L.current_stream(dev)), "mf_compact_mask")
    n = int(count.item())
    return (oa[:n] if oa is not None else None), (ob[:n] if ob is not None else None)


def _pass_stats(p, N):
    dev = p["alphas"].device
    lib = L.lib()
    d = L.mf_loss_pass()
    d.alphas, d.disp_local, d.disp_global = L.ptr(p["alphas"]), L.ptr(p.get("disp_local")), L.ptr(p.get("disp_global"))
    d.n_samples = p["alphas"].shape[1]
    out = torch.empty(12, dtype=torch.float64, device=dev)
    means = torch.empty(6, dtype=torch.float32, device=dev)
    scratch = torch.empty(int(lib.mf_loss_partials_scratch_bytes()), dtype=torch.uint8, device=dev)
    with torch.cuda.device(dev):
        L.check(lib.mf_loss_partials(C.byref(d), None, None, N, out.data_ptr(), means.data_ptr(), scratch.data_ptr(),
                                     L.current_stream(dev)), "mf_loss_partials")
    return {"local": (out[4], out[5], means[2]), "global": (out[8], out[9], means[4]), "out12": out}


def _consensus_vectors(p, N, loc, glob):
    if not LAZY_CONSENSUS:
        return _compact(p["alphas"], p.get("disp_local"), p.get("disp_global"))
    from .lazy import ConsensusPass, MaskedVector

    def compact():
        la, ga = _compact(p["alphas"], p.get("disp_local"), p.get("disp_global"))
        return {"local": la, "global": ga}

    g = ConsensusPass(p["alphas"], {"local": p.get("disp_local"), "global": p.get("disp_global")}, lambda: _pass_stats(p, N), compact,
                      differentiable=False)
    return (MaskedVector(g, "local") if loc else None), (MaskedVector(g, "global") if glob else None)


def sample_pdf(bins, weights, N_importance, det=False, eps=1e-5):
    L.require_gpu(bins, "sample_pdf")
    dev = bins.device
    N, nb = bins.shape
    if weights.shape != (N, nb - 1):
        raise RuntimeError(f"sample_pdf: weights must be (N, {nb - 1}), got {tuple(weights.shape)}")
    M = N_importance
    if det:
        u, u_stride = _linspace01(M, dev), 0
    else:
        u, u_stride = torch.rand(N, M, device=dev), M
    b = bins.detach().contiguous().float()
    w = weights.detach().contiguous().float()
    out = torch.empty((N, M), device=dev, dtype=torch.float32)
    with torch.cuda.device(dev):
        L.check(L.lib().mf_sample_pdf_eps(L.ptr(b), None, L.ptr(w), nb - 1, N, nb, M, L.ptr(u), u_stride, None,
                                          L.ptr(out), None, None, float(eps), L.current_stream(dev)), "mf_sample_pdf")
    return out


def resample_merge(z_vals, weights, N_importance, det=True, u=None, return_aux=False, cdf=None):
    L.require_gpu(z_vals, "resample_merge")
    dev = z_vals.device
    N, S = z_vals.shape
    M = N_importance
    if u is None:
        if det:
            u = _linspace01(M, dev)
            u_stride = 0
        else:
            u = torch.rand(N, M, device=dev)
            u_stride = M
    else:
        u = u.contiguous().float()
        u_stride = M if u.dim() == 2 else 0
    if cdf is not None:
        cdf = cdf.detach().contiguous().float()
    z = z_vals.detach().contiguous().float()
    w = weights.detach().contiguous().float()
    z_out = torch.empty((N, S + M), device=dev, dtype=torch.float32)
    inds = torch.empty((N, M), device=dev, dtype=torch.int32) if return_aux else None
    z_new = torch.empty((N, M), device=dev, dtype=torch.float32) if return_aux else None
    with torch.cuda.device(dev):
        L.check(L.lib().mf_sample_pdf(None, L.ptr(z), w.data_ptr() + 4, S, N, S - 1, M, L.ptr(u), u_stride,
                                      L.ptr(cdf), L.ptr(z_new), L.ptr(inds), L.ptr(z_out),
                                      L.current_stream(dev)), "mf_sample_pdf")
    if return_aux:
        return z_out, inds, z_new
    return z_out


def render_rays(rays,
                background,
                nerf_embeddings,
                nerf_models,
                nof_embeddings=None,
                nof_models=None,
                chain_local=False,
                chain_global=False,
                N_samples=64,
                N_importance=0,
                use_disp=False,
                perturb=0,
                noise_std=1,
                nerf_activate_type='relu',
                test_time=False,
                _capture=None,
                _rng=None,
                _loss_target=None,
                ):
    _rng = _rng or {}
    L.require_gpu(rays, "render_rays")
    if nerf_activate_type == 'relu':
        act = L.MF_ACT_RELU
    elif nerf_activate_type == 'softplus':
        act = L.MF_ACT_SOFTPLUS
    else:
        raise ValueError('activation layer type: %s not support' % nerf_activate_type)
    use_nof = nof_models is not None
    if use_nof and chain_global and not chain_local and not test_time:
        raise UnboundLocalError("local variable 'fw_nof' referenced before assignment")
    all_models = list(nerf_models) + (list(nof_models) if use_nof else [])
    grad = A.needs_grad(all_models)
    dev = rays.device
    rays = rays.detach().float()
    if rays.dim() != 2 or rays.shape[1] < (10 if (use_nof and chain_global) else 9):
        raise RuntimeError(f"render_rays: rays must be (N, 9|10), got {tuple(rays.shape)}")
    if rays.stride(1) != 1:
        rays = rays.contiguous()
    if background is not None:
        background = background.detach().float().contiguous()
    N = rays.shape[0]
    S = N_samples
    loc = bool(use_nof and chain_local and not test_time)
    glob = bool(use_nof and chain_global and not test_time)
    need_fine = N_importance > 0

    z_steps = _linspace01(S, dev)
    z_vals = None
    if perturb > 0 or need_fine or grad:
        pr = None
        if perturb > 0:
            pr = _rng["perturb_rand"] if "perturb_rand" in _rng else torch.rand((N, S), device=dev)
            pr = pr.contiguous().float()
        z_vals = torch.empty((N, S), device=dev, dtype=torch.float32)
        with torch.cuda.device(dev):
            L.check(L.lib().mf_z_vals(L.ptr(rays), rays.stride(0), N, L.ptr(z_steps), S, 1 if use_disp else 0,
                                      L.ptr(pr), float(perturb), L.ptr(z_vals), L.current_stream(dev)), "mf_z_vals")

    def draw_noise(shape, key=None):
        if key in _rng:
            return _rng[key].contiguous().float()
        if noise_std != 0:
            return (torch.randn(shape, device=dev) * noise_std).contiguous()
        if STRICT_RNG and shape[0] > 0:
            torch.randn(shape, device=dev)
        return None

    coarse_opacity_only = bool(need_fine and test_time)
    coarse_sigma_only = coarse_opacity_only and not grad
    pass_prec = TRAIN_FORWARD_PRECISION if grad else None
    want_planes = need_fine or loc or glob or grad or _capture is not None
    noise_c = draw_noise((N, S), "noise_coarse")
    if grad and N > 0:
        if coarse_opacity_only and _loss_target is not None:
            raise NotImplementedError("render_rays(test_time=True, N_importance > 0, _loss_target=...) with gradients: the fused loss "
                                      "partials need rgb_coarse, which a test_time pass does not return")
        for m in nerf_models[:2 if need_fine else 1]:
            A.require_nerf_hip(m, N * S, use_nof)
        if use_nof:
            for m in nof_models:
                A.require_nof_hip(m, nof_embeddings)
    ws = [None]
    c = _render_pass(rays, background, z_vals, None if z_vals is not None else z_steps, use_disp,
                     noise_c, act, nerf_models[0], nerf_embeddings,
                     nof_models if use_nof else None, nof_embeddings, loc, glob, coarse_sigma_only, want_planes,
                     dump=grad and not coarse_sigma_only, precision=pass_prec, workspace=ws)
    if coarse_opacity_only:
        result = {'opacity_coarse': c["opacity"]}
    else:
        result = {'rgb_coarse': c["rgb"], 'depth_coarse': c["depth"], 'opacity_coarse': c["opacity"]}
    fused_loss = _loss_target is not None
    training = grad and N > 0
    if (loc or glob) and not fused_loss:
        la, ga = (None, None) if training else _consensus_vectors(c, N, loc, glob)
        if loc:
            result['nof_local_disp_coarse'] = la
        if glob:
            result['nof_global_disp_coarse'] = ga

    if _capture is not None:
        _capture.update(z_coarse=z_vals, weights_coarse=c.get("weights"), alphas_coarse=c.get("alphas"))
    if need_fine:
        z_all = resample_merge(z_vals, c["weights"], N_importance, det=(perturb == 0), u=_rng.get("u"))
        noise_f = draw_noise((N, S + N_importance), "noise_fine")
        f = _render_pass(rays, background, z_all, None, use_disp, noise_f, act,
                         nerf_models[1], nerf_embeddings, nof_models if use_nof else None, nof_embeddings,
                         loc, glob, False, loc or glob or grad or _capture is not None,
                         dump=grad, precision=pass_prec, workspace=ws)
        if _capture is not None:
            _capture.update(z_fine=z_all, weights_fine=f.get("weights"), alphas_fine=f.get("alphas"))
        result['rgb_fine'] = f["rgb"]
        result['depth_fine'] = f["depth"]
        result['opacity_fine'] = f["opacity"]
        if (loc or glob) and not fused_loss:
            la, ga = (None, None) if training else _consensus_vectors(f, N, loc, glob)
            if loc:
                result['nof_local_disp_fine'] = la
            if glob:
                result['nof_global_disp_fine'] = ga
    if fused_loss and not (grad and N > 0):
        result['loss_partials'] = _loss_partials_hip(c, f if need_fine else None, _loss_target, N)
    if grad and N > 0:
        result = _attach_explicit(result, rays, background, nerf_embeddings, nerf_models, nof_embeddings,
                                  nof_models if use_nof else None, loc, glob, nerf_activate_type,
                                  (c, z_vals, noise_c), (f, z_all, noise_f) if need_fine else None,
                                  loss_target=_loss_target, coarse_opacity_only=coarse_opacity_only)
    return result


def _attach_explicit(result, rays, background, nerf_embs, nerf_models, nof_embs, nof_models, loc, glob,
                     activation, coarse, fine, loss_target=None, coarse_opacity_only=False):
    rays_o, rays_d, ind = rays[:, 0:3], rays[:, 3:6], rays[:, 8:9]
    out, recons, kernel_vals = {}, {}, set()

    def one(tag, nerf, pack, opacity_only=False):
        p, z, noise = pack
        N, S = z.shape
        xyz = rays_o.unsqueeze(1) + rays_d.unsqueeze(1) * z.unsqueeze(2)
        group = None
        if (loc or glob) and loss_target is None:
            from .lazy import ConsensusPass, MaskedVector
            planes, recon_of = {}, {}
            group = ConsensusPass(p["alphas"], planes, lambda: _pass_stats(p, N),
                                  lambda g: {k: torch.masked_select(g.plane(k), _mask_of(p["alphas"])) for k in planes}, True,
                                  mean_fn=(lambda g, k: A.ConsensusMean.apply(g, k, p, rays, z, recon_of[k])) if FUSED_CONSENSUS_MEAN else None,
                                  pass_self=True)

            def vector(key, recon):
                recon_of[key] = recon
                planes[key] = lambda: torch.abs(xyz - recon).mean(-1)
                v = MaskedVector(group, key)
                return v if LAZY_CONSENSUS else v.materialize()
        xin = p["xyz_in"]
        if nof_models is not None:
            bw = nof_models[0]
            if "nof_acts" in p:
                step = [0]
                plane = p["nof_plane"]
                if p.get("nof_emb") is None:
                    p["nof_emb"] = _nof_embedded_inputs(p, plane, xyz.detach().reshape(-1, 3), rays, S, nof_embs)
                n_bw = sum(1 for k in range(len(plane)) if k in (0, 3))
                batched = (N * S) % 128 == 0 and (len(nof_models) < 2 or nof_models[0] is not nof_models[1])
                trains = lambda m: any(q.requires_grad for q in m.parameters())
                sinks = {}
                slots = not getattr(p["nof_emb"], "_mf_natural", False)
                if batched and trains(bw):
                    sinks[id(bw)] = (A.NofGradSink(bw, p["nof_acts"][:n_bw], p["nof_emb"][:n_bw], slots), 0)
                if batched and len(plane) > n_bw and trains(nof_models[1]):
                    sinks[id(nof_models[1])] = (A.NofGradSink(nof_models[1], p["nof_acts"][n_bw:], p["nof_emb"][n_bw:], slots), n_bw)
                gated = {key: A.NofParamGate.apply(sk, *sk.m.parameters()) for key, (sk, _) in sinks.items()}

                def nof_points(pts, ray_ind, embs_, m):
                    k = plane[step[0]]
                    step[0] += 1
                    sk, first = sinks.get(id(m), (None, 0))
                    emb_k = p["nof_emb"][k]
                    emb_k._mf_natural = not slots
                    return A.nof_points_dumped(pts, nof_embs, m, p["nof_acts"][k], emb_k, p["nof_out"][k],
                                               sink=sk, sink_plane=k - first, params=gated.get(id(m)))
            else:
                nof_points = A.nof_points
            canon = nof_points(xyz, ind, nof_embs, bw)
            if loc:
                fw = nof_models[1]
                recon = nof_points(canon, ind, nof_embs, fw)
                if loss_target is None:
                    out[f"nof_local_disp_{tag}"] = vector("local", recon)
                else:
                    recons[f"local_{tag}"] = recon
            if glob:
                cind = rays[:, 9:10]
                a_ = nof_points(canon, cind, nof_embs, fw)
                b_ = nof_points(a_, cind, nof_embs, bw)
                chained = nof_points(b_, ind, nof_embs, fw)
                if loss_target is None:
                    out[f"nof_global_disp_{tag}"] = vector("global", chained)
                else:
                    recons[f"global_{tag}"] = chained
            xin = canon.reshape(-1, 3)
        with torch.no_grad():
            emb_in = nerf_embs[0].rows(p["xyz_in"], 1, max(64, nerf.in_channels_xyz))
            extra_in = None
            if nerf.extra_feat_type == "ind":
                extra_in = nerf_embs[1].rows(ind, S, max(32, nerf.extra_feat_dim))
            elif nerf.extra_feat_type == "dir":
                extra_in = nerf_embs[2].rows(rays_d, S, max(32, nerf.extra_feat_dim))
        rgbsig = A.NerfSamples.apply(nerf, p["acts"], p["rgbsig"], emb_in, extra_in, nerf_embs[0], xin, opacity_only,
                                     *nerf.parameters())
        if S > 2048:
            raise NotImplementedError(f"render_rays with gradients: mf_composite_backward is built for <= 2048 samples per ray, got {S}")
        out[f"rgb_{tag}"], out[f"depth_{tag}"], out[f"opacity_{tag}"] = A.CompositeSamples.apply(
            rgbsig, rays, z, noise, activation, background, p["rgb"], p["depth"], p["opacity"])
        kernel_vals.update((f"rgb_{tag}", f"depth_{tag}", f"opacity_{tag}"))

    one("coarse", nerf_models[0], coarse, opacity_only=coarse_opacity_only)
    if fine is not None:
        one("fine", nerf_models[1], fine)
    final = {}
    for k, v in result.items():
        t = out[k]
        final[k] = t if (k in kernel_vals or v is None) else v.detach() + (t - t.detach())
    if loss_target is not None:
        tgt = loss_target.detach().float().contiguous()
        passes = [dict(planes=coarse[0], z=coarse[1])] + ([dict(planes=fine[0], z=fine[1])] if fine is not None else [])
        tensors = []
        for tag in ("coarse", "fine")[:len(passes)]:
            tensors += [out[f"rgb_{tag}"], recons.get(f"local_{tag}"), recons.get(f"global_{tag}")]
        N = rays.shape[0]
        final["loss_partials"] = A.LossPartials.apply(
            lambda: _loss_partials_hip(coarse[0], fine[0] if fine is not None else None, tgt, N), rays, tgt, passes, *tensors)
    return final


def _nof_embedded_inputs(p, plane, x_obs, rays, S, nof_embs):
    steps, P = len(plane), x_obs.shape[0]
    out_of = lambda k: p["nof_out"][plane[k]]
    src = {0: x_obs, 1: out_of(0), 2: out_of(0)}
    if steps > 3:
        src[3], src[4] = out_of(2), out_of(3)
    if steps == 2:
        src = {0: x_obs, 1: out_of(0)}
    emb = torch.empty((steps, P, 80), device=x_obs.device, dtype=torch.float32)
    ex = nof_embs[0].descriptor()
    with torch.no_grad():
        ind_i = nof_embs[1](rays[:, 8:9].contiguous())
        ind_j = nof_embs[1](rays[:, 9:10].contiguous()) if steps > 2 else None
    with torch.cuda.device(x_obs.device):
        for k in range(steps):
            tab = ind_j if k in (2, 3) else ind_i
            pts = src[k].contiguous()
            L.check(L.lib().mf_nof_embed_rows(ex, L.ptr(pts), L.ptr(tab), tab.shape[1], S, P, emb[plane[k]].data_ptr(),
                                              L.current_stream(x_obs.device)), "mf_nof_embed_rows")
    emb._mf_natural = True
    return emb


def _mask_of(alphas):
    mask = alphas.ge(0.01)
    if not torch.any(mask):
        mask = torch.ones_like(mask).bool()
    return mask
```

Measured before the change: 121.2 million.

## Fold NeRF final linear layer into the extra-encoding layer weights

The NeRF trunk's final layer (xyz_encoding_final, linear with no activation) is folded into the following extra_encoding layer by precomputing W_extra_hidden·W_final and the combined bias in double precision at pack time. A new render kernel variant skips that 256x256 layer and goes straight from the last trunk layer to the extra layer. This removes one full dense layer per sample from the render path. It is gated on fp32, W=256 and no dump, and it changes rounding slightly because the product is computed ahead of time.

```diff
diff --git a/include/mocoflow_hip.h b/include/mocoflow_hip.h
--- a/include/mocoflow_hip.h
+++ b/include/mocoflow_hip.h
@@ -67,6 +67,8 @@
 int64_t mf_nof_packed_bytes_p(const mf_nof_desc* d, int32_t precision);
 int32_t mf_nerf_pack_p(const mf_nerf_desc* d, int32_t precision, void* packed, void* stream);
 int32_t mf_nof_pack_p(const mf_nof_desc* d, int32_t precision, void* packed, void* stream);
+int64_t mf_nerf_fold_packed_bytes(const mf_nerf_desc* d);
+int32_t mf_nerf_pack_fold(const mf_nerf_desc* d, void* packed, void* stream);
 
 int32_t mf_embedding_forward(const mf_embedding* e, const float* x, int64_t B, float* out, void* stream);
 int32_t mf_embedding_forward_rows(const mf_embedding* e, const float* x, int64_t B, int32_t repeat, float* out,
@@ -154,7 +156,8 @@
 enum {
   MF_F_SIGMA_ONLY   = 1 << 0,
   MF_F_CHAIN_LOCAL  = 1 << 1,
-  MF_F_CHAIN_GLOBAL = 1 << 2
+  MF_F_CHAIN_GLOBAL = 1 << 2,
+  MF_F_FOLDED_FINAL = 1 << 3
 };
 
 typedef struct mf_render_args {
diff --git a/moco_flow_amd/_lib.py b/moco_flow_amd/_lib.py
--- a/moco_flow_amd/_lib.py
+++ b/moco_flow_amd/_lib.py
@@ -8,7 +8,7 @@
 MF_MAX_LAYERS = 16
 MF_EXTRA_NONE, MF_EXTRA_IND, MF_EXTRA_DIR = 0, 1, 2
 MF_ACT_RELU, MF_ACT_SOFTPLUS = 0, 1
-MF_F_SIGMA_ONLY, MF_F_CHAIN_LOCAL, MF_F_CHAIN_GLOBAL = 1, 2, 4
+MF_F_SIGMA_ONLY, MF_F_CHAIN_LOCAL, MF_F_CHAIN_GLOBAL, MF_F_FOLDED_FINAL = 1, 2, 4, 8
 MF_PREC_F32, MF_PREC_BF16, MF_PREC_BF16X3 = 0, 1, 2
 PRECISIONS = {"f32": MF_PREC_F32, "bf16": MF_PREC_BF16, "bf16x3": MF_PREC_BF16X3}
 MF_ABI_VERSION = 16
@@ -125,6 +125,8 @@
     "mf_nof_forward": (C.c_int32, [C.POINTER(mf_nof_desc), _fp, _fp, C.c_int64, _fp, C.c_int64, _fp, _fp]),
     "mf_nerf_bwd_packed_bytes": (C.c_int64, [C.POINTER(mf_nerf_desc)]),
     "mf_nerf_pack_bwd": (C.c_int32, [C.POINTER(mf_nerf_desc), _fp, _fp]),
+    "mf_nerf_fold_packed_bytes": (C.c_int64, [C.POINTER(mf_nerf_desc)]),
+    "mf_nerf_pack_fold": (C.c_int32, [C.POINTER(mf_nerf_desc), _fp, _fp]),
     "mf_nof_points_dump": (C.c_int32, [C.POINTER(mf_nof_desc), _fp, C.POINTER(mf_embedding), C.POINTER(mf_embedding), _fp, _fp,
                                        C.c_int64, C.c_int32, C.c_int64, _fp, _fp, C.c_int64, _fp, _fp]),
     "mf_nof_forward_dump": (C.c_int32, [C.POINTER(mf_nof_desc), _fp, _fp, C.c_int64, _fp, C.c_int64, _fp, _fp, C.c_int64, _fp]),
diff --git a/moco_flow_amd/csrc/mf_layout.hpp b/moco_flow_amd/csrc/mf_layout.hpp
--- a/moco_flow_amd/csrc/mf_layout.hpp
+++ b/moco_flow_amd/csrc/mf_layout.hpp
@@ -111,6 +111,21 @@
   return true;
 }
 
+struct FoldLayout {
+  int64_t panel_bytes;
+  int64_t scratch_bytes;
+  int64_t off_w, off_b;
+};
+inline bool nerf_fold_layout(const mf_nerf_desc& d, NetLayout& L, FoldLayout& F) {
+  F = FoldLayout{};
+  if (!nerf_layout(d, L, 0) || L.W != 256) return false;
+  F.panel_bytes = L.panel_bytes - (int64_t)trunk_groups(L, L.n_trunk - 1) * L.NP * kGroupBytes;
+  F.scratch_bytes = round_up(((int64_t)(L.W / 2) * L.W + L.W / 2) * 4, kGroupBytes);
+  F.off_w = L.res_bytes + F.panel_bytes;
+  F.off_b = F.off_w + (int64_t)(L.W / 2) * L.W * 4;
+  return true;
+}
+
 inline bool nof_layout(const mf_nof_desc& d, NetLayout& L, int bf16 = 0, bool wide_ok = false) {
   L = NetLayout{};
   const bool x3 = bf16 == MF_PREC_BF16X3;
diff --git a/moco_flow_amd/csrc/mf_nets.hpp b/moco_flow_amd/csrc/mf_nets.hpp
--- a/moco_flow_amd/csrc/mf_nets.hpp
+++ b/moco_flow_amd/csrc/mf_nets.hpp
@@ -18,6 +18,14 @@
   f.groups = trunk_groups(n.L, layer);
   f.jump = nullptr;
   f.bias_off = n.res_lds + (n.L.off_bias_trunk + layer * n.L.W) * 4;
+  return f;
+}
+
+MF_D NextLayer next_extra(const NetDev& n) {
+  NextLayer f;
+  f.groups = extra_groups(n.L);
+  f.jump = nullptr;
+  f.bias_off = n.res_lds + n.L.off_bias_extra * 4;
   return f;
 }
 
@@ -86,7 +94,7 @@
   }
 }
 
-template <int NK, bool DUMP = false>
+template <int NK, bool DUMP = false, bool FOLD = false>
 MF_D void nerf_eval(const NetDev& net, const float (&embx)[kStepsNerfXyz], const float (&ext)[kStepsExtraMax],
                     bool sigma_only, Stream& st, CarryT<kPD>& carry, const LaneId& id,
                     const NextLayer& follow, float& sigma, float (&rgb)[3], float* dump_row = nullptr,
@@ -96,10 +104,12 @@
   for (int t = 0; t < NK; ++t)
 #pragma unroll
     for (int i = 0; i < 4; ++i) act[t][i] = 0;
+  static_assert(!(FOLD && DUMP), "the dump rows hold xyz_encoding_final's output");
   const int D = net.L.n_trunk - 1;
   for (int l = 0; l < D; ++l) {
     const bool last = sigma_only && l == D - 1;
-    trunk_layer<NK, kStepsNerfXyz, DUMP>(net, l, act, embx, st, carry, id, last ? follow : next_trunk(net, l + 1),
+    trunk_layer<NK, kStepsNerfXyz, DUMP>(net, l, act, embx, st, carry, id,
+                                               last ? follow : ((FOLD && l == D - 1) ? next_extra(net) : next_trunk(net, l + 1)),
                                                dump_row ? dump_row + l * net.L.W : nullptr, mask_row ? mask_row + l * 8 : nullptr);
     st.tl.stamp(10 + l, id);
   }
@@ -108,12 +118,11 @@
   sigma = sg[0];
   st.tl.stamp(30, id);
   if (sigma_only) return;
-  NextLayer ex;
-  ex.groups = extra_groups(net.L);
-  ex.jump = nullptr;
-  ex.bias_off = net.res_lds + net.L.off_bias_extra * 4;
-  trunk_layer<NK, kStepsNerfXyz, DUMP>(net, D, act, embx, st, carry, id, ex,
-                                             dump_row ? dump_row + D * net.L.W : nullptr);
+  if constexpr (!FOLD) {
+    const NextLayer ex = next_extra(net);
+    trunk_layer<NK, kStepsNerfXyz, DUMP>(net, D, act, embx, st, carry, id, ex,
+                                               dump_row ? dump_row + D * net.L.W : nullptr);
+  }
   st.tl.stamp(31, id);
   f32x4 e[NK / 2];
   extra_layer<NK, DUMP>(net, act, ext, e, st, carry, id, follow, dump_row ? dump_row + (D + 1) * net.L.W : nullptr,
diff --git a/moco_flow_amd/csrc/mf_pack.hip b/moco_flow_amd/csrc/mf_pack.hip
--- a/moco_flow_amd/csrc/mf_pack.hip
+++ b/moco_flow_amd/csrc/mf_pack.hip
@@ -111,6 +111,27 @@
   job.dst[(e * kNofIndCols + c) * job.rows + r] = c < job.cols ? job.scale * job.W[e][(long long)r * job.n_in[e] + job.col0 + c] : 0.f;
 }
 
+struct FoldJob { const float *We, *Wf, *be, *bf; int W, ld_e; float *Wp, *bp; };
+
+__global__ void fold_final_kernel(FoldJob job) {
+  const int idx = blockIdx.x * blockDim.x + threadIdx.x;
+  const int half = job.W / 2;
+  if (idx >= half * job.W) return;
+  const int n = idx / job.W, k = idx % job.W;
+  const float* we = job.We + (long long)n * job.ld_e;
+  double acc = 0.0;
+  for (int j = 0; j < job.W; ++j) acc += (double)we[j] * (double)job.Wf[(long long)j * job.W + k];
+  job.Wp[idx] = (float)acc;
+  if (idx < half) {
+    const float* wb = job.We + (long long)idx * job.ld_e;
+    double b = 0.0;
+#ifndef MF_FOLD_BREAK_BIAS
+    for (int j = 0; j < job.W; ++j) b += (double)wb[j] * (double)job.bf[j];
+#endif
+    job.bp[idx] = (float)((double)job.be[idx] + b);
+  }
+}
+
 int launch_pack(const PackJob& job, hipStream_t st, const char* what) {
   const long long slots = job.total_groups * 64 > job.res_floats ? job.total_groups * 64 : job.res_floats;
   hipLaunchKernelGGL(pack_panels_kernel, dim3((unsigned)((slots + 255) / 256)), dim3(256), 0, st, job);
@@ -138,12 +159,17 @@
   return L.res_bytes + L.panel_bytes + L.ind_bytes;
 }
 
-extern "C" int32_t mf_nerf_pack_p(const mf_nerf_desc* d, int32_t precision, void* packed, void* stream) {
-  NetLayout L;
+static int32_t nerf_pack(const mf_nerf_desc* d, int32_t precision, void* packed, void* stream, bool fold) {
+  NetLayout L;
+  FoldLayout F{};
   if (!d || !packed) return fail(MF_E_INVALID, "mf_nerf_pack: null argument");
   if (precision < MF_PREC_F32 || precision > MF_PREC_BF16X3) return fail(MF_E_INVALID, "mf_nerf_pack: precision %d", precision);
-  if (!nerf_layout(*d, L, precision)) return fail(MF_E_UNSUPPORTED, "mf_nerf_pack: unsupported NeRF configuration "
+  if (fold ? !nerf_fold_layout(*d, L, F) : !nerf_layout(*d, L, precision))
+    return fail(MF_E_UNSUPPORTED, "mf_nerf_pack: unsupported NeRF configuration "
                                        "(W=%d D=%d in_channels_xyz=%d)", d->W, d->D, d->in_channels_xyz);
+  const int64_t panel_bytes = fold ? F.panel_bytes : L.panel_bytes;
+  float* const fold_w = fold ? reinterpret_cast<float*>(static_cast<char*>(packed) + F.off_w) : nullptr;
+  float* const fold_b = fold ? reinterpret_cast<float*>(static_cast<char*>(packed) + F.off_b) : nullptr;
   PackJob job{};
   ResJob rj{};
   const int esplit = L.emb_split ? L.terms : 1, equad = L.bf16 ? 1 : 4;
@@ -160,6 +186,7 @@
     const bool has_emb = (L.emb_mask >> l) & 1;
     const float* W = l < d->D ? d->trunk_w[l] : d->final_w;
     if (!W) return fail(MF_E_INVALID, "mf_nerf_pack: missing weight pointer for layer %d", l);
+    if (fold && l == d->D) continue;
     const int hid0 = has_emb ? d->in_channels_xyz : 0, n_in = hid0 + (l > 0 ? L.W : 0);
     job.add(L.NP, trunk_groups(L, l),
             PackBlock{W, n_in, 1, kEmbNerfXyz, has_emb ? L.emb_steps / equad : 0, esplit, d->in_channels_xyz},
@@ -173,9 +200,11 @@
     if (!W) return fail(MF_E_INVALID, "mf_nerf_pack: missing extra_encoding weight");
     const int kind = d->extra_feat_type == MF_EXTRA_DIR ? kEmbDir : (d->extra_feat_type == MF_EXTRA_IND ? kEmbInd : kEmbNone);
     job.add(L.NP / 2, extra_groups(L),
-            PackBlock{W, L.W + ext, 1, kPackHidden, hidden_batches(L), ((L.hsplit_mask >> L.n_trunk) & 1) ? L.terms : 1, L.W},
+            fold ? PackBlock{fold_w, L.W, 1, kPackHidden, hidden_batches(L), 1, L.W}
+                 : PackBlock{W, L.W + ext, 1, kPackHidden, hidden_batches(L), ((L.hsplit_mask >> L.n_trunk) & 1) ? L.terms : 1, L.W},
             PackBlock{W + L.W, L.W + ext, 1, kind, L.extra_steps / equad, esplit, ext});
-    rj.c[rj.n++] = ResCopy{d->extra_b, L.off_bias_extra, L.W / 2};
+    if (fold && (!d->extra_b || !d->final_b)) return fail(MF_E_INVALID, "mf_nerf_pack: missing bias pointer of the folded layers");
+    rj.c[rj.n++] = ResCopy{fold ? fold_b : d->extra_b, L.off_bias_extra, L.W / 2};
   }
   if (L.head_tiles) {
     if (!d->rgb_w) return fail(MF_E_INVALID, "mf_nerf_pack: missing rgb weight");
@@ -192,8 +221,29 @@
   job.panels = reinterpret_cast<float*>(static_cast<char*>(packed) + L.res_bytes);
   rj.res = static_cast<float*>(packed);
   rj.total = (int)(L.res_bytes / 4);
-  if (job.total_groups * kGroupBytes != L.panel_bytes) return fail(MF_E_INVALID, "mf_nerf_pack: layout mismatch");
+  if (job.total_groups * kGroupBytes != panel_bytes) return fail(MF_E_INVALID, "mf_nerf_pack: layout mismatch");
+  if (fold) {
+    const int ext = d->extra_feat_type == MF_EXTRA_NONE ? 0 : d->extra_feat_dim;
+    const FoldJob fj{d->extra_w, d->final_w, d->extra_b, d->final_b, L.W, L.W + ext, fold_w, fold_b};
+    hipLaunchKernelGGL(fold_final_kernel, dim3((L.W / 2) * L.W / 256), dim3(256), 0, static_cast<hipStream_t>(stream), fj);
+    if (int e = check_launch("mf_nerf_pack_fold")) return e;
+  }
   return launch_pack(job, rj, static_cast<hipStream_t>(stream));
+}
+
+extern "C" int32_t mf_nerf_pack_p(const mf_nerf_desc* d, int32_t precision, void* packed, void* stream) {
+  return nerf_pack(d, precision, packed, stream, false);
+}
+
+extern "C" int64_t mf_nerf_fold_packed_bytes(const mf_nerf_desc* d) {
+  NetLayout L;
+  FoldLayout F;
+  if (!d || !nerf_fold_layout(*d, L, F)) { fail(MF_E_UNSUPPORTED, "mf_nerf_fold_packed_bytes: unsupported NeRF configuration (fp32, W = 256)"); return 0; }
+  return L.res_bytes + F.panel_bytes + F.scratch_bytes;
+}
+
+extern "C" int32_t mf_nerf_pack_fold(const mf_nerf_desc* d, void* packed, void* stream) {
+  return nerf_pack(d, MF_PREC_F32, packed, stream, true);
 }
 
 extern "C" int32_t mf_nof_pack_p(const mf_nof_desc* d, int32_t precision, void* packed, void* stream) {
diff --git a/moco_flow_amd/csrc/mf_render.hip b/moco_flow_amd/csrc/mf_render.hip
--- a/moco_flow_amd/csrc/mf_render.hip
+++ b/moco_flow_amd/csrc/mf_render.hip
@@ -33,169 +33,14 @@
 
 template <bool MOCO, bool DUMP>
 __global__ __launch_bounds__(kThreads, 2) void render_kernel(RenderParams p) {
-  const LaneId id;
-  const NetDev nerf = p.nerf;
-  const WgClock wg;
-  load_resident(nerf, id);
-  if (MOCO) {
-    load_resident(p.bw, id);
-    if (p.flags & (MF_F_CHAIN_LOCAL | MF_F_CHAIN_GLOBAL)) load_resident(p.fw, id);
-  }
-  emb_tables_to_lds(p);
-  const uint32_t par_nerf_xyz = p.par_off, par_nerf_ext = p.par_off + 128, par_nof_xyz = p.par_off + 256,
-                 par_nof_ind = p.par_off + 384;
-  Stream st;
-  CarryT<kPD> carry;
-  st.open(p.ring_off, p.buf_bytes, MF_TIMING_FLAGS ? p.dbg : 0);
-  st.tl.start(p.alphas, id);
-  const NextLayer prog_first = MOCO ? follow_of(p.bw) : follow_of(nerf);
-  if (MOCO) start_program(p.bw, st, carry, id);
-  else start_program(nerf, st, carry, id);
+  constexpr bool FOLD = false;
+#include "mf_render_body.hpp"
+}
 
-  const int S = p.S;
-  const bool sigma_only = p.flags & MF_F_SIGMA_ONLY;
-  float4* sbuf = reinterpret_cast<float4*>(smem + p.sbuf_off);
-  float* zbuf = reinterpret_cast<float*>(smem + p.zbuf_off);
-
-  for (long long group = blockIdx.x; group < p.n_groups; group += gridDim.x) {
-    const long long ray0 = group * p.G;
-    const int nr = (int)((p.n_rays - ray0) < p.G ? (p.n_rays - ray0) : p.G);
-    const int nsamp = nr * S;
-    const int ntiles = (nsamp + kTile - 1) / kTile;
-
-    for (int tile = 0; tile < ntiles; ++tile) {
-      st.tl.stamp(1, id);
-      struct Where { int srel, sl, si; bool valid; long long ray; const float* rp; };
-      auto where = [&]() {
-        int jo = id.j;
-        asm volatile("" : "+v"(jo));
-        Where w;
-        w.srel = tile * kTile + id.wave * kWaveSamples + jo;
-        w.valid = w.srel < nsamp;
-        w.sl = w.valid ? w.srel : nsamp - 1;
-        const int rr = w.sl / S;
-        w.si = w.sl - rr * S;
-        w.ray = ray0 + rr;
-        w.rp = p.rays + w.ray * p.ray_stride;
-        return w;
-      };
-      float xin[3];
-      {
-        const Where w = where();
-        const float* rp = w.rp;
-        const float o[3] = {rp[0], rp[1], rp[2]};
-        const float d[3] = {rp[3], rp[4], rp[5]};
-        const float z = ray_depth(p, rp, w.ray, w.si);
-        ray_point(o, d, z, xin);
-        if (w.valid && id.g == 0) {
-          zbuf[w.srel] = z;
-          if (MOCO) sbuf[w.srel] = make_float4(xin[0], xin[1], xin[2], 0.f);
-        }
-      }
-#ifdef MF_TIMELINE
-      asm volatile("s_waitcnt vmcnt(0)" : "+v"(xin[0]), "+v"(xin[1]), "+v"(xin[2]));
-#endif
-      st.tl.stamp(2, id);
-      if (MOCO) {
-        const int nsteps = chain_steps(p.flags);
-        float canon[3] = {0.f, 0.f, 0.f}, cur[3] = {xin[0], xin[1], xin[2]};
-        for (int step = 0; step < nsteps; ++step) {
-          const int role = step;
-          const NetDev net = role_uses_fw(role) ? p.fw : p.bw;
-          const Where w = where();
-          const float ind = w.rp[role_ind_column(role)];
-          if (role == 1 || role == 2) { cur[0] = canon[0]; cur[1] = canon[1]; cur[2] = canon[2]; }
-          const bool last = step == nsteps - 1;
-          const NextLayer follow = last ? follow_of(nerf) : (role_uses_fw(role + 1) ? follow_of(p.fw) : follow_of(p.bw));
-          float emb[kStepsNofIn], out[3];
-          nof_embed_lds(emb, cur, ind, par_nof_xyz, par_nof_ind, id.g);
-          float* nof_row = nullptr;
-          if constexpr (DUMP) {
-            if (w.valid && p.dump_nof_acts) {
-              const long long nof_idx = (long long)((p.nof_plane_pack >> (3 * step)) & 7u) * p.n_rays * S + (w.ray * S + w.si);
-              nof_row = p.dump_nof_acts + nof_idx * p.dump_nof_stride;
-              float4* e4 = reinterpret_cast<float4*>(p.dump_nof_emb + nof_idx * 80 + 20 * id.g);
-#pragma unroll
-              for (int q = 0; q < kStepsNofIn / 4; ++q) e4[q] = make_float4(emb[4 * q], emb[4 * q + 1], emb[4 * q + 2], emb[4 * q + 3]);
-            }
-            st.keep2 = 0;
-          }
-          nof_eval<DUMP>(net, emb, cur, st, carry, id, follow, out, nof_row,
-                         DUMP && p.dump_nof_stride >= (long long)net.L.n_trunk * net.L.W + 16 + 4 * net.L.n_trunk);
-          if constexpr (DUMP) {
-            const Where v = where();
-            if (v.valid && p.dump_nof_acts && id.g == 0) {
-              const long long nof_idx = (long long)((p.nof_plane_pack >> (3 * step)) & 7u) * p.n_rays * S + (v.ray * S + v.si);
-              float* q = p.dump_nof_out + nof_idx * 3;
-              q[0] = out[0]; q[1] = out[1]; q[2] = out[2];
-            }
-          }
-          if (role == 0) { canon[0] = out[0]; canon[1] = out[1]; canon[2] = out[2]; }
-          if (role == 1 || role == 4) {
-            const Where v = where();
-            const float4 x4 = sbuf[v.sl];
-            const float dd = (fabsf(x4.x - out[0]) + fabsf(x4.y - out[1]) + fabsf(x4.z - out[2])) / 3.f;
-            float* plane = role == 1 ? p.disp_local : p.disp_global;
-            if (v.valid && id.g == 0 && plane) plane[v.ray * S + v.si] = dd;
-          }
-          cur[0] = out[0]; cur[1] = out[1]; cur[2] = out[2];
-        }
-        xin[0] = canon[0]; xin[1] = canon[1]; xin[2] = canon[2];
-      }
-
-      st.tl.stamp(3, id);
-      float embx[kStepsNerfXyz], ext[kStepsExtraMax];
-      if (!(MF_TIMING_FLAGS && (p.dbg & 4))) emb_eval_lds<3, 10>(embx, xin, par_nerf_xyz, id.g);
-      else { for (int e = 0; e < kStepsNerfXyz; ++e) embx[e] = xin[e % 3]; }
-#pragma unroll
-      for (int e = BlkXyz10::SLOTS; e < kStepsNerfXyz; ++e) embx[e] = 0.f;
-#pragma unroll
-      for (int e = 0; e < kStepsExtraMax; ++e) ext[e] = 0.f;
-      float* dump_row = nullptr;
-      unsigned* mask_row = nullptr;
-      {
-        const Where w = where();
-        if (!sigma_only) {
-          if (p.extra_type == MF_EXTRA_DIR) {
-            const float dd[3] = {w.rp[3], w.rp[4], w.rp[5]};
-            emb_eval_lds<3, 4>(ext, dd, par_nerf_ext, id.g);
-          } else if (p.extra_type == MF_EXTRA_IND) {
-            const float iv[1] = {w.rp[8]};
-            emb_eval_lds<1, 2>(ext, iv, par_nerf_ext, id.g);
-          }
-        }
-        if constexpr (DUMP) {
-          if (w.valid && p.dump_acts) dump_row = p.dump_acts + (w.ray * S + w.si) * p.dump_stride;
-          if (p.dump_mask) mask_row = p.dump_mask + (w.ray * S + w.si) * p.dump_mask_stride;
-        }
-      }
-      st.tl.stamp(4, id);
-      float sigma, rgb[3] = {0.f, 0.f, 0.f};
-      st.keep2 = 0;
-      nerf_eval<16, DUMP>(nerf, embx, ext, sigma_only, st, carry, id, prog_first, sigma, rgb, dump_row, mask_row);
-      {
-        const Where w = where();
-        if (w.valid && id.g == 0) {
-          sbuf[w.srel] = make_float4(rgb[0], rgb[1], rgb[2], sigma);
-          if constexpr (DUMP) {
-            const long long row = w.ray * S + w.si;
-            if (p.dump_rgbsigma) *reinterpret_cast<float4*>(p.dump_rgbsigma + row * 4) = make_float4(rgb[0], rgb[1], rgb[2], sigma);
-            if (p.dump_xyz) { float* q = p.dump_xyz + row * 3; q[0] = xin[0]; q[1] = xin[1]; q[2] = xin[2]; }
-          }
-        }
-      }
-      st.tl.stamp(5, id);
-    }
-    __syncthreads();
-    st.tl.stamp(6, id);
-
-    composite_group<kWaves>(p, id.lane, id.wave, ray0, (MF_TIMING_FLAGS && (p.dbg & 8)) ? 0 : nr, S, sigma_only, sbuf, zbuf);
-    st.tl.stamp(7, id);
-    __syncthreads();
-    st.tl.stamp(8, id);
-  }
-  wait_vm0();
-  wg.stamp(p);
+template <bool MOCO>
+__global__ __launch_bounds__(kThreads, 2) void render_fold_kernel(RenderParams p) {
+  constexpr bool DUMP = false, FOLD = true;
+#include "mf_render_body.hpp"
 }
 
 int render_pass_bf16(const mf_render_args* a, hipStream_t st, bool prepare_only);
@@ -229,6 +74,12 @@
   const bool dump = a->dump_acts || a->dump_rgbsigma || a->dump_xyz || a->dump_nof_acts;
   if (dump && a->precision == MF_PREC_BF16)
     return fail(MF_E_UNSUPPORTED, "mf_render_pass: the activation dump (training forward) exists in fp32 and in bf16x3");
+  if (a->flags & MF_F_FOLDED_FINAL) {
+    if (a->precision != MF_PREC_F32)
+      return fail(MF_E_UNSUPPORTED, "mf_render_pass: MF_F_FOLDED_FINAL is built for MF_PREC_F32 (precision %d)", a->precision);
+    if (dump || a->dump_mask || a->dump_nof_emb || a->dump_nof_out)
+      return fail(MF_E_INVALID, "mf_render_pass: MF_F_FOLDED_FINAL with a dump_* pointer (the training forward reads mf_nerf_pack's stream)");
+  }
   if (int e = check_xyz_embedding("mf_render_pass", a->emb_xyz, 10)) return e;
   const bool sigma_only = a->flags & MF_F_SIGMA_ONLY;
   if (!sigma_only && a->nerf->extra_feat_type == MF_EXTRA_DIR &&
@@ -296,6 +147,7 @@
   const bool dump = a->dump_acts || a->dump_rgbsigma || a->dump_xyz || a->dump_nof_acts;
   void (*kern)(RenderParams) =
       dump ? (moco ? render_kernel<true, true> : render_kernel<false, true>)
+           : (a->flags & MF_F_FOLDED_FINAL) ? (moco ? render_fold_kernel<true> : render_fold_kernel<false>)
            : (moco ? render_kernel<true, false> : render_kernel<false, false>);
   return launch_lds(kern, persistent_grid(p.n_groups), kThreads, lds, st, p, "mf_render_pass", "mf_render_pass");
 }
diff --git a/moco_flow_amd/csrc/mf_render_body.hpp b/moco_flow_amd/csrc/mf_render_body.hpp
--- /dev/null
+++ b/moco_flow_amd/csrc/mf_render_body.hpp
@@ -0,0 +1,163 @@
+  const LaneId id;
+  const NetDev nerf = p.nerf;
+  const WgClock wg;
+  load_resident(nerf, id);
+  if (MOCO) {
+    load_resident(p.bw, id);
+    if (p.flags & (MF_F_CHAIN_LOCAL | MF_F_CHAIN_GLOBAL)) load_resident(p.fw, id);
+  }
+  emb_tables_to_lds(p);
+  const uint32_t par_nerf_xyz = p.par_off, par_nerf_ext = p.par_off + 128, par_nof_xyz = p.par_off + 256,
+                 par_nof_ind = p.par_off + 384;
+  Stream st;
+  CarryT<kPD> carry;
+  st.open(p.ring_off, p.buf_bytes, MF_TIMING_FLAGS ? p.dbg : 0);
+  st.tl.start(p.alphas, id);
+  const NextLayer prog_first = MOCO ? follow_of(p.bw) : follow_of(nerf);
+  if (MOCO) start_program(p.bw, st, carry, id);
+  else start_program(nerf, st, carry, id);
+
+  const int S = p.S;
+  const bool sigma_only = p.flags & MF_F_SIGMA_ONLY;
+  float4* sbuf = reinterpret_cast<float4*>(smem + p.sbuf_off);
+  float* zbuf = reinterpret_cast<float*>(smem + p.zbuf_off);
+
+  for (long long group = blockIdx.x; group < p.n_groups; group += gridDim.x) {
+    const long long ray0 = group * p.G;
+    const int nr = (int)((p.n_rays - ray0) < p.G ? (p.n_rays - ray0) : p.G);
+    const int nsamp = nr * S;
+    const int ntiles = (nsamp + kTile - 1) / kTile;
+
+    for (int tile = 0; tile < ntiles; ++tile) {
+      st.tl.stamp(1, id);
+      struct Where { int srel, sl, si; bool valid; long long ray; const float* rp; };
+      auto where = [&]() {
+        int jo = id.j;
+        asm volatile("" : "+v"(jo));
+        Where w;
+        w.srel = tile * kTile + id.wave * kWaveSamples + jo;
+        w.valid = w.srel < nsamp;
+        w.sl = w.valid ? w.srel : nsamp - 1;
+        const int rr = w.sl / S;
+        w.si = w.sl - rr * S;
+        w.ray = ray0 + rr;
+        w.rp = p.rays + w.ray * p.ray_stride;
+        return w;
+      };
+      float xin[3];
+      {
+        const Where w = where();
+        const float* rp = w.rp;
+        const float o[3] = {rp[0], rp[1], rp[2]};
+        const float d[3] = {rp[3], rp[4], rp[5]};
+        const float z = ray_depth(p, rp, w.ray, w.si);
+        ray_point(o, d, z, xin);
+        if (w.valid && id.g == 0) {
+          zbuf[w.srel] = z;
+          if (MOCO) sbuf[w.srel] = make_float4(xin[0], xin[1], xin[2], 0.f);
+        }
+      }
+#ifdef MF_TIMELINE
+      asm volatile("s_waitcnt vmcnt(0)" : "+v"(xin[0]), "+v"(xin[1]), "+v"(xin[2]));
+#endif
+      st.tl.stamp(2, id);
+      if (MOCO) {
+        const int nsteps = chain_steps(p.flags);
+        float canon[3] = {0.f, 0.f, 0.f}, cur[3] = {xin[0], xin[1], xin[2]};
+        for (int step = 0; step < nsteps; ++step) {
+          const int role = step;
+          const NetDev net = role_uses_fw(role) ? p.fw : p.bw;
+          const Where w = where();
+          const float ind = w.rp[role_ind_column(role)];
+          if (role == 1 || role == 2) { cur[0] = canon[0]; cur[1] = canon[1]; cur[2] = canon[2]; }
+          const bool last = step == nsteps - 1;
+          const NextLayer follow = last ? follow_of(nerf) : (role_uses_fw(role + 1) ? follow_of(p.fw) : follow_of(p.bw));
+          float emb[kStepsNofIn], out[3];
+          nof_embed_lds(emb, cur, ind, par_nof_xyz, par_nof_ind, id.g);
+          float* nof_row = nullptr;
+          if constexpr (DUMP) {
+            if (w.valid && p.dump_nof_acts) {
+              const long long nof_idx = (long long)((p.nof_plane_pack >> (3 * step)) & 7u) * p.n_rays * S + (w.ray * S + w.si);
+              nof_row = p.dump_nof_acts + nof_idx * p.dump_nof_stride;
+              float4* e4 = reinterpret_cast<float4*>(p.dump_nof_emb + nof_idx * 80 + 20 * id.g);
+#pragma unroll
+              for (int q = 0; q < kStepsNofIn / 4; ++q) e4[q] = make_float4(emb[4 * q], emb[4 * q + 1], emb[4 * q + 2], emb[4 * q + 3]);
+            }
+            st.keep2 = 0;
+          }
+          nof_eval<DUMP>(net, emb, cur, st, carry, id, follow, out, nof_row,
+                         DUMP && p.dump_nof_stride >= (long long)net.L.n_trunk * net.L.W + 16 + 4 * net.L.n_trunk);
+          if constexpr (DUMP) {
+            const Where v = where();
+            if (v.valid && p.dump_nof_acts && id.g == 0) {
+              const long long nof_idx = (long long)((p.nof_plane_pack >> (3 * step)) & 7u) * p.n_rays * S + (v.ray * S + v.si);
+              float* q = p.dump_nof_out + nof_idx * 3;
+              q[0] = out[0]; q[1] = out[1]; q[2] = out[2];
+            }
+          }
+          if (role == 0) { canon[0] = out[0]; canon[1] = out[1]; canon[2] = out[2]; }
+          if (role == 1 || role == 4) {
+            const Where v = where();
+            const float4 x4 = sbuf[v.sl];
+            const float dd = (fabsf(x4.x - out[0]) + fabsf(x4.y - out[1]) + fabsf(x4.z - out[2])) / 3.f;
+            float* plane = role == 1 ? p.disp_local : p.disp_global;
+            if (v.valid && id.g == 0 && plane) plane[v.ray * S + v.si] = dd;
+          }
+          cur[0] = out[0]; cur[1] = out[1]; cur[2] = out[2];
+        }
+        xin[0] = canon[0]; xin[1] = canon[1]; xin[2] = canon[2];
+      }
+
+      st.tl.stamp(3, id);
+      float embx[kStepsNerfXyz], ext[kStepsExtraMax];
+      if (!(MF_TIMING_FLAGS && (p.dbg & 4))) emb_eval_lds<3, 10>(embx, xin, par_nerf_xyz, id.g);
+      else { for (int e = 0; e < kStepsNerfXyz; ++e) embx[e] = xin[e % 3]; }
+#pragma unroll
+      for (int e = BlkXyz10::SLOTS; e < kStepsNerfXyz; ++e) embx[e] = 0.f;
+#pragma unroll
+      for (int e = 0; e < kStepsExtraMax; ++e) ext[e] = 0.f;
+      float* dump_row = nullptr;
+      unsigned* mask_row = nullptr;
+      {
+        const Where w = where();
+        if (!sigma_only) {
+          if (p.extra_type == MF_EXTRA_DIR) {
+            const float dd[3] = {w.rp[3], w.rp[4], w.rp[5]};
+            emb_eval_lds<3, 4>(ext, dd, par_nerf_ext, id.g);
+          } else if (p.extra_type == MF_EXTRA_IND) {
+            const float iv[1] = {w.rp[8]};
+            emb_eval_lds<1, 2>(ext, iv, par_nerf_ext, id.g);
+          }
+        }
+        if constexpr (DUMP) {
+          if (w.valid && p.dump_acts) dump_row = p.dump_acts + (w.ray * S + w.si) * p.dump_stride;
+          if (p.dump_mask) mask_row = p.dump_mask + (w.ray * S + w.si) * p.dump_mask_stride;
+        }
+      }
+      st.tl.stamp(4, id);
+      float sigma, rgb[3] = {0.f, 0.f, 0.f};
+      st.keep2 = 0;
+      nerf_eval<16, DUMP, FOLD>(nerf, embx, ext, sigma_only, st, carry, id, prog_first, sigma, rgb, dump_row, mask_row);
+      {
+        const Where w = where();
+        if (w.valid && id.g == 0) {
+          sbuf[w.srel] = make_float4(rgb[0], rgb[1], rgb[2], sigma);
+          if constexpr (DUMP) {
+            const long long row = w.ray * S + w.si;
+            if (p.dump_rgbsigma) *reinterpret_cast<float4*>(p.dump_rgbsigma + row * 4) = make_float4(rgb[0], rgb[1], rgb[2], sigma);
+            if (p.dump_xyz) { float* q = p.dump_xyz + row * 3; q[0] = xin[0]; q[1] = xin[1]; q[2] = xin[2]; }
+          }
+        }
+      }
+      st.tl.stamp(5, id);
+    }
+    __syncthreads();
+    st.tl.stamp(6, id);
+
+    composite_group<kWaves>(p, id.lane, id.wave, ray0, (MF_TIMING_FLAGS && (p.dbg & 8)) ? 0 : nr, S, sigma_only, sbuf, zbuf);
+    st.tl.stamp(7, id);
+    __syncthreads();
+    st.tl.stamp(8, id);
+  }
+  wait_vm0();
+  wg.stamp(p);
diff --git a/moco_flow_amd/nerf.py b/moco_flow_amd/nerf.py
--- a/moco_flow_amd/nerf.py
+++ b/moco_flow_amd/nerf.py
@@ -39,6 +39,7 @@
         self._packed_x3 = PackedWeights()
         self._packed_bwd3 = PackedWeights()
         self._packed_bwd = PackedWeights()
+        self._packed_fold = PackedWeights()
 
     def _build_desc(self):
         if self.extra_feat_type == "latent_code":
@@ -76,8 +77,13 @@
         return cache.get(self, self._build_desc, lib.mf_nerf_packed_bytes_p, lib.mf_nerf_pack_p, "NeRF", precision)
 
     def invalidate_packed(self):
-        for c in (self._packed, self._packed_bf16, self._packed_x3, self._packed_bwd, self._packed_bwd3):
+        for c in (self._packed, self._packed_bf16, self._packed_x3, self._packed_bwd, self._packed_bwd3, self._packed_fold):
             c.invalidate()
+
+    def packed_fold(self):
+        lib = L.lib()
+        return self._packed_fold.get(self, self._build_desc, lambda d, _p: lib.mf_nerf_fold_packed_bytes(d),
+                                     lambda d, _p, buf, st: lib.mf_nerf_pack_fold(d, buf, st), "NeRF (folded final layer)", "fold")
 
     def packed_bwd(self):
         lib = L.lib()
diff --git a/moco_flow_amd/rendering.py b/moco_flow_amd/rendering.py
--- a/moco_flow_amd/rendering.py
+++ b/moco_flow_amd/rendering.py
@@ -1,6 +1,7 @@
 from __future__ import annotations
 
 import ctypes as C
+import os
 
 import torch
 
@@ -10,6 +11,9 @@
 
 PRECISION = "f32"
 TRAIN_FORWARD_PRECISION = "f32"
+
+
+FOLD_FINAL = os.environ.get("MF_FOLD_FINAL", "1") != "0"
 
 
 def set_train_forward_precision(p: str):
@@ -83,10 +87,14 @@
         flags |= L.MF_F_CHAIN_LOCAL
     if chain_global:
         flags |= L.MF_F_CHAIN_GLOBAL
-    a.flags = flags
     prec = L.PRECISIONS[precision or PRECISION]
     a.precision = prec
-    desc, buf = nerf.packed(prec)
+    if FOLD_FINAL and prec == L.MF_PREC_F32 and not dump and nerf.W == 256:
+        flags |= L.MF_F_FOLDED_FINAL
+        desc, buf = nerf.packed_fold()
+    else:
+        desc, buf = nerf.packed(prec)
+    a.flags = flags
     a.nerf, a.nerf_packed = C.pointer(desc), buf.data_ptr()
     a.emb_xyz = _emb_desc(nerf_embs[0])
     if nerf.extra_feat_type == "ind":
```

New measurement: 136.2 million, median of 6. 1.12x the previous value.
